# freewym/espresso

Measured on AMD Instinct MI355X. Metric: audio-hours/sec training (LibriSpeech Conformer-12 + CTC), higher is better.
Workload: dtype bf16; 1 GPU; LibriSpeech 960h Conformer-12 + CTC update step, <=26000 frames & <=24 utts per GPU, V=5004, on-GPU fbank+CMVN+SpecAugment, dropout 0.1, clip 2.0, Adam; parallelism=dp1

## Files before the change

espresso_amd/criterions/ctc_loss.py:

```python
import math

import torch

from .. import functional as F
from ..registry import register_criterion


@register_criterion("ctc_loss")
class CtcLossCriterion:
    def __init__(self, task, sentence_avg=True, zero_infinity=True, print_training_sample_interval=500):
        self.task = task
        d = task.target_dictionary
        if hasattr(task, "blank_symbol"):
            if task.blank_symbol is None:
                raise ValueError(f"{type(self).__name__} needs task.blank_symbol (task.criterion_name must name this criterion)")
            self.blank_idx = d.index(task.blank_symbol)
        else:
            self.blank_idx = d.bos()
        self.pad_idx = d.pad()
        self.eos_idx = d.eos()
        self.sentence_avg = sentence_avg
        self.zero_infinity = zero_infinity
        self.print_interval = print_training_sample_interval
        self.num_updates = -1
        self.epoch = 0

    def set_num_updates(self, num_updates):
        self.num_updates = num_updates

    def set_epoch(self, epoch):
        self.epoch = epoch

    def __call__(self, model, sample, reduce=True):
        return self.forward(model, sample, reduce)

    def forward(self, model, sample, reduce=True):
        net_output = model(**sample["net_input"], **({"epoch": self.epoch} if False else {}))
        input_lengths = net_output["src_lengths"][0]
        target = sample["target"]
        pad_mask = (target != self.pad_idx) & (target != self.eos_idx)
        target_lengths = pad_mask.sum(-1)
        lg = net_output.get("_logits_bt")
        if lg:
            logits = lg[0]
            B, Tp = net_output["encoder_padding_mask"][0].shape
        else:
            e = net_output["encoder_out"][0]
            Tp, B, V = e.shape
            logits = e.transpose(0, 1).reshape(B * Tp, V)
        nll, lprobs = F.ctc_loss(logits, target.to(torch.int32).contiguous(), input_lengths.to(torch.int32).contiguous(),
                                 target_lengths.to(torch.int32).contiguous(), B, Tp, blank=self.blank_idx,
                                 zero_infinity=self.zero_infinity)
        if self.zero_infinity:
            nll = torch.where(torch.isinf(nll), torch.zeros_like(nll), nll)
        loss = nll.sum()
        ntokens = sample["ntokens"] if "ntokens" in sample else int(target_lengths.sum())
        nsentences = target.size(0)
        sample_size = nsentences if self.sentence_avg else ntokens
        logging_output = {
            "loss": loss.detach(),
            "ntokens": ntokens,
            "nsentences": nsentences,
            "sample_size": sample_size,
        }
        return loss, sample_size, logging_output

    @staticmethod
    def reduce_metrics(logging_outputs):
        loss_sum = float(sum(float(l.get("loss", 0)) for l in logging_outputs))
        ntokens = sum(l.get("ntokens", 0) for l in logging_outputs)
        nsentences = sum(l.get("nsentences", 0) for l in logging_outputs)
        sample_size = sum(l.get("sample_size", 0) for l in logging_outputs)
        out = {"loss": loss_sum / max(sample_size, 1) / math.log(2), "ntokens": ntokens, "nsentences": nsentences,
               "sample_size": sample_size}
        if sample_size != ntokens:
            out["nll_loss"] = loss_sum / max(ntokens, 1) / math.log(2)
        return out

    @staticmethod
    def logging_outputs_can_be_summed():
        return True
```

espresso_amd/csrc/elementwise.hip:

```cpp
#include "common.h"
#include "espresso_amd.h"

namespace {

__global__ __launch_bounds__(256) void cast_f32_bf16_kernel(const float* __restrict__ src,
                                                            bf16_t* __restrict__ dst, long n) {
  const long stride = (long)gridDim.x * blockDim.x * 8;
  for (long i = ((long)blockIdx.x * blockDim.x + threadIdx.x) * 8; i < n; i += stride) {
    if (i + 8 <= n) {
      const float4 a = *reinterpret_cast<const float4*>(src + i);
      const float4 b = *reinterpret_cast<const float4*>(src + i + 4);
      uint4 u;
      u.x = pack_bf2(a.x, a.y);
      u.y = pack_bf2(a.z, a.w);
      u.z = pack_bf2(b.x, b.y);
      u.w = pack_bf2(b.z, b.w);
      *reinterpret_cast<uint4*>(dst + i) = u;
    } else {
      for (long j = i; j < n; ++j) dst[j] = f2bf(src[j]);
    }
  }
}

__global__ __launch_bounds__(256) void cast_f32_bf16_rows_kernel(const float* __restrict__ src, long ld_src, bf16_t* __restrict__ dst,
                                                                 long ld_dst, int N) {
  const long m = blockIdx.y;
  const float* s = src + m * ld_src;
  bf16_t* d = dst + m * ld_dst;
  const bool vec = (ld_src & 3) == 0 && (ld_dst & 7) == 0 && ((reinterpret_cast<uintptr_t>(src) | reinterpret_cast<uintptr_t>(dst)) & 15) == 0;
  for (int n = (blockIdx.x * 256 + threadIdx.x) * 8; n < ld_dst; n += gridDim.x * 256 * 8) {
    if (vec && n + 8 <= N) {
      const float4 a = *reinterpret_cast<const float4*>(s + n);
      const float4 b = *reinterpret_cast<const float4*>(s + n + 4);
      uint4 u;
      u.x = pack_bf2(a.x, a.y);
      u.y = pack_bf2(a.z, a.w);
      u.z = pack_bf2(b.x, b.y);
      u.w = pack_bf2(b.z, b.w);
      *reinterpret_cast<uint4*>(d + n) = u;
    } else {
      for (int j = n; j < n + 8 && j < ld_dst; ++j) d[j] = j < N ? f2bf(s[j]) : (bf16_t)0;
    }
  }
}

__global__ __launch_bounds__(256) void cast_bf16_f32_kernel(const bf16_t* __restrict__ src,
                                                            float* __restrict__ dst, long n) {
  const long stride = (long)gridDim.x * blockDim.x;
  for (long i = (long)blockIdx.x * blockDim.x + threadIdx.x; i < n; i += stride) dst[i] = bf2f(src[i]);
}

__global__ __launch_bounds__(256) void scale_dropout_kernel(const bf16_t* __restrict__ x,
                                                            const bf16_t* __restrict__ y,
                                                            bf16_t* __restrict__ out, long n, float a,
                                                            float b, uint64_t seed, uint32_t thr,
                                                            float inv_keep) {
  const long stride = (long)gridDim.x * blockDim.x * 8;
  for (long i = ((long)blockIdx.x * blockDim.x + threadIdx.x) * 8; i < n; i += stride) {
    if (i + 8 <= n) {
      const uint4 ux = *reinterpret_cast<const uint4*>(x + i);
      uint4 uy = make_uint4(0, 0, 0, 0);
      if (y) uy = *reinterpret_cast<const uint4*>(y + i);
      const uint32_t wx[4] = {ux.x, ux.y, ux.z, ux.w};
      const uint32_t wy[4] = {uy.x, uy.y, uy.z, uy.w};
      float o[8], k8[8];
      if (thr) ea_keep8(seed, (uint64_t)i, thr, inv_keep, k8);
#pragma unroll
      for (int e = 0; e < 8; ++e) {
        const float xv = (e & 1) ? __uint_as_float(wx[e >> 1] & 0xffff0000u) : __uint_as_float(wx[e >> 1] << 16);
        const float yv = (e & 1) ? __uint_as_float(wy[e >> 1] & 0xffff0000u) : __uint_as_float(wy[e >> 1] << 16);
        const float k = thr ? k8[e] : 1.f;
        o[e] = a * xv * k + b * yv;
      }
      uint4 u;
      u.x = pack_bf2(o[0], o[1]);
      u.y = pack_bf2(o[2], o[3]);
      u.z = pack_bf2(o[4], o[5]);
      u.w = pack_bf2(o[6], o[7]);
      *reinterpret_cast<uint4*>(out + i) = u;
    } else {
      for (long j = i; j < n; ++j) {
        float k = 1.f;
        if (thr) k = ea_keep(seed, (uint64_t)j, thr, inv_keep);
        out[j] = f2bf(a * bf2f(x[j]) * k + b * (y ? bf2f(y[j]) : 0.f));
      }
    }
  }
}

__global__ __launch_bounds__(256) void colsum_kernel(const bf16_t* __restrict__ X, float* __restrict__ out,
                                                     int M, int N, long ld, int rows_per_block) {
  __shared__ float sm[8][64];
  const int cx = threadIdx.x & 31, ry = threadIdx.x >> 5;
  const int c0 = blockIdx.x * 64 + cx * 2;
  const int r0 = blockIdx.y * rows_per_block;
  const int r1 = min(M, r0 + rows_per_block);
  float a0 = 0.f, a1 = 0.f;
  if (c0 + 1 < N && (ld & 1) == 0) {
    for (int r = r0 + ry; r < r1; r += 8) {
      const uint32_t w = *reinterpret_cast<const uint32_t*>(X + (long)r * ld + c0);
      a0 += __uint_as_float(w << 16);
      a1 += __uint_as_float(w & 0xffff0000u);
    }
  } else {
    for (int r = r0 + ry; r < r1; r += 8) {
      if (c0 < N) a0 += bf2f(X[(long)r * ld + c0]);
      if (c0 + 1 < N) a1 += bf2f(X[(long)r * ld + c0 + 1]);
    }
  }
  sm[ry][cx * 2] = a0;
  sm[ry][cx * 2 + 1] = a1;
  __syncthreads();
  if (threadIdx.x < 64) {
    float s = 0.f;
#pragma unroll
    for (int i = 0; i < 8; ++i) s += sm[i][threadIdx.x];
    const int c = blockIdx.x * 64 + threadIdx.x;
    if (c < N) atomicAdd(out + c, s);
  }
}

__global__ __launch_bounds__(256) void zero_rows_kernel(bf16_t* __restrict__ x, const uint8_t* __restrict__ row_zero,
                                                        int M, int C) {
  const int row = blockIdx.x;
  if (!row_zero[row]) return;
  for (int c = threadIdx.x; c < C; c += 256) x[(long)row * C + c] = 0;
}

__global__ __launch_bounds__(256) void embedding_fwd_kernel(const int* __restrict__ tok, const int* __restrict__ position,
                                                            const float* __restrict__ W, const float* __restrict__ pos,
                                                            bf16_t* __restrict__ out, int M, int C, float scale) {
  const int row = blockIdx.x * 4 + (threadIdx.x >> 6);
  if (row >= M) return;
  const float* w = W + (long)tok[row] * C;
  const float* pe = pos ? pos + (long)position[row] * C : nullptr;
  for (int c = (threadIdx.x & 63) * 2; c < C; c += 128) {
    float a = scale * w[c], b = scale * w[c + 1];
    if (pe) { a += pe[c]; b += pe[c + 1]; }
    *reinterpret_cast<uint32_t*>(out + (long)row * C + c) = pack_bf2(a, b);
  }
}
__global__ __launch_bounds__(256) void embedding_bwd_kernel(const int* __restrict__ tok, const bf16_t* __restrict__ dy,
                                                            float* __restrict__ dW, int M, int C, float scale, int pad_idx) {
  const int row = blockIdx.x * 4 + (threadIdx.x >> 6);
  if (row >= M) return;
  const int t = tok[row];
  if (t == pad_idx) return;
  float* w = dW + (long)t * C;
  for (int c = (threadIdx.x & 63); c < C; c += 64) atomicAdd(w + c, scale * bf2f(dy[(long)row * C + c]));
}

}

static inline int grid_for(long n, int per_thread) {
  long b = (n + 256L * per_thread - 1) / (256L * per_thread);
  if (b > 4096) b = 4096;
  if (b < 1) b = 1;
  return (int)b;
}

struct TransposeBatch {
  const bf16_t* src[8];
  bf16_t* dst[8];
  int rows[8], cols[8], tile0[9];
  int n;
};
__global__ __launch_bounds__(256) void transpose_batch_kernel(const TransposeBatch tb) {
  __shared__ bf16_t tile[64][66];
  int mi = 0;
#pragma unroll
  for (int i = 1; i < 8; ++i)
    if (i < tb.n && (int)blockIdx.x >= tb.tile0[i]) mi = i;
  const int R = tb.rows[mi], Cc = tb.cols[mi];
  const int tcols = (Cc + 63) / 64;
  const int t = blockIdx.x - tb.tile0[mi];
  const int r0 = (t / tcols) * 64, c0 = (t % tcols) * 64;
  const bf16_t* __restrict__ src = tb.src[mi];
  bf16_t* __restrict__ dst = tb.dst[mi];
  const int tx = threadIdx.x & 63, ty = threadIdx.x >> 6;
  for (int i = ty; i < 64; i += 4)
    if (r0 + i < R && c0 + tx < Cc) tile[i][tx] = src[(long)(r0 + i) * Cc + c0 + tx];
  __syncthreads();
  for (int i = ty; i < 64; i += 4)
    if (c0 + i < Cc && r0 + tx < R) dst[(long)(c0 + i) * R + r0 + tx] = tile[tx][i];
}

extern "C" int ea_transpose_bf16_batch(const void* const* src, void* const* dst, const int* rows, const int* cols, int n,
                                       hipStream_t stream) {
  if (n <= 0) return 0;
  if (n > 8) return -2;
  TransposeBatch tb;
  int tot = 0;
  for (int i = 0; i < 8; ++i) {
    tb.src[i] = i < n ? (const bf16_t*)src[i] : nullptr;
    tb.dst[i] = i < n ? (bf16_t*)dst[i] : nullptr;
    tb.rows[i] = i < n ? rows[i] : 0;
    tb.cols[i] = i < n ? cols[i] : 0;
    tb.tile0[i] = tot;
    if (i < n) tot += ((rows[i] + 63) / 64) * ((cols[i] + 63) / 64);
  }
  tb.tile0[8] = tot;
  tb.n = n;
  if (tot == 0) return 0;
  hipLaunchKernelGGL(transpose_batch_kernel, dim3(tot), dim3(256), 0, stream, tb);
  return EA_CHECK_LAUNCH();
}

extern "C" int ea_cast_f32_to_bf16(const float* src, void* dst, long n, hipStream_t stream) {
  if (n <= 0) return 0;
  hipLaunchKernelGGL(cast_f32_bf16_kernel, dim3(grid_for(n, 8)), dim3(256), 0, stream, src, (bf16_t*)dst, n);
  return EA_CHECK_LAUNCH();
}
extern "C" int ea_cast_f32_to_bf16_rows(const float* src, long ld_src, void* dst, long ld_dst, long M, int N, hipStream_t stream) {
  if (M <= 0 || N <= 0) return 0;
  if (ld_dst < N || ld_src < N || M > 65535) return -2;
  const int bx = (int)((ld_dst + 2047) / 2048);
  hipLaunchKernelGGL(cast_f32_bf16_rows_kernel, dim3(bx, (unsigned)M), dim3(256), 0, stream, src, ld_src, (bf16_t*)dst, ld_dst, N);
  return EA_CHECK_LAUNCH();
}
extern "C" int ea_cast_bf16_to_f32(const void* src, float* dst, long n, hipStream_t stream) {
  if (n <= 0) return 0;
  hipLaunchKernelGGL(cast_bf16_f32_kernel, dim3(grid_for(n, 1)), dim3(256), 0, stream, (const bf16_t*)src, dst, n);
  return EA_CHECK_LAUNCH();
}
extern "C" int ea_dropout_hash_host(uint64_t seed, uint64_t idx0, long n, uint32_t* out) {
  if (!out || n < 0) return -1;
  for (long i = 0; i < n; ++i) out[i] = ea_hash(seed, idx0 + (uint64_t)i);
  return 0;
}
extern "C" int ea_scale_dropout_bf16(const void* x, const void* y, void* out, long n, float a, float b,
                                     uint64_t seed, uint32_t thr, float inv_keep, hipStream_t stream) {
  if (n <= 0) return 0;
  hipLaunchKernelGGL(scale_dropout_kernel, dim3(grid_for(n, 8)), dim3(256), 0, stream, (const bf16_t*)x,
                     (const bf16_t*)y, (bf16_t*)out, n, a, b, seed, thr, inv_keep);
  return EA_CHECK_LAUNCH();
}
extern "C" int ea_colsum_bf16(const void* X, float* out, int M, int N, long ld, hipStream_t stream) {
  if (M <= 0 || N <= 0) return 0;
  int rpb = (M + 255) / 256;
  if (rpb < 64) rpb = 64;
  dim3 grid((N + 63) / 64, (M + rpb - 1) / rpb);
  hipLaunchKernelGGL(colsum_kernel, grid, dim3(256), 0, stream, (const bf16_t*)X, out, M, N, ld, rpb);
  return EA_CHECK_LAUNCH();
}
extern "C" int ea_zero_rows_bf16(void* x, const uint8_t* row_zero, int M, int C, hipStream_t stream) {
  if (M <= 0) return 0;
  hipLaunchKernelGGL(zero_rows_kernel, dim3(M), dim3(256), 0, stream, (bf16_t*)x, row_zero, M, C);
  return EA_CHECK_LAUNCH();
}

extern "C" int ea_embedding_fwd(const int* tokens, const int* positions, const float* W, const float* pos_table, void* out,
                                int M, int C, float scale, hipStream_t stream) {
  if (M <= 0) return 0;
  if (C % 2) return -2;
  hipLaunchKernelGGL(embedding_fwd_kernel, dim3((M + 3) / 4), dim3(256), 0, stream, tokens, positions, W, pos_table, (bf16_t*)out, M, C, scale);
  return EA_CHECK_LAUNCH();
}
extern "C" int ea_embedding_bwd(const int* tokens, const void* dy, float* dW, int M, int C, float scale, int pad_idx,
                                hipStream_t stream) {
  if (M <= 0) return 0;
  hipLaunchKernelGGL(embedding_bwd_kernel, dim3((M + 3) / 4), dim3(256), 0, stream, tokens, (const bf16_t*)dy, dW, M, C, scale, pad_idx);
  return EA_CHECK_LAUNCH();
}
```

espresso_amd/csrc/loss.hip:

```cpp
#include "common.h"
#include "espresso_amd.h"
#include "softmax_row.h"

namespace {

template <typename TIn>
__global__ __launch_bounds__(256) void log_softmax_kernel(const TIn* __restrict__ in, long ld_in,
                                                          float* __restrict__ out, int V) {
  __shared__ float sm[16];
  const long row = blockIdx.x;
  const TIn* x = in + row * ld_in;
  const float lse = log_softmax_row_lse<TIn, false>(x, V, sm);
  log_softmax_row_write<TIn, false>(x, V, lse, out + row * (long)V);
}

__device__ __forceinline__ int ctc_label(const int* tg, int s, int blank) { return (s & 1) ? tg[s >> 1] : blank; }

__global__ __launch_bounds__(256) void ctc_gather_kernel(const float* __restrict__ lprobs, const int* __restrict__ targets,
                                                         const int* __restrict__ in_len, const int* __restrict__ tgt_len,
                                                         float* __restrict__ G, int T, int V, int Lmax, int blank) {
  const int b = blockIdx.y, t = blockIdx.x;
  if (t >= in_len[b]) return;
  const int S = 2 * tgt_len[b] + 1, Smax = 2 * Lmax + 1;
  const float* lp = lprobs + ((long)b * T + t) * V;
  const int* tg = targets + (long)b * Lmax;
  float* g = G + ((long)b * T + t) * Smax;
  for (int s = threadIdx.x; s < S; s += blockDim.x) g[s] = lp[ctc_label(tg, s, blank)];
}

__global__ void ctc_scan_kernel(const float* __restrict__ G, const int* __restrict__ targets,
                                const int* __restrict__ in_len, const int* __restrict__ tgt_len,
                                float* __restrict__ A, float* __restrict__ Bt, float* __restrict__ nll_out,
                                int T, int Lmax, int blank, int SP) {
  extern __shared__ float sh[];
  const int b = blockIdx.x;
  const int Tb = in_len[b], L = tgt_len[b];
  const int S = 2 * L + 1, Smax = 2 * Lmax + 1;
  const int dir = blockIdx.y;
  const int s = threadIdx.x;
  float* buf0 = sh + 0 * (SP + 2) + (dir ? 0 : 2);
  float* buf1 = sh + 1 * (SP + 2) + (dir ? 0 : 2);
  const int* tg = targets + (long)b * Lmax;
  if (Tb <= 0) {
    if (threadIdx.x == 0 && dir == 0) nll_out[b] = (L == 0) ? 0.f : INFINITY;
    return;
  }
  bool skip = false;
  if (s < S) {
    if (!dir) { if ((s & 1) && s >= 2) skip = tg[s >> 1] != tg[(s >> 1) - 1]; }
    else      { if ((s & 1) && s + 2 < S) skip = tg[(s >> 1) + 1] != tg[s >> 1]; }
  }
  if (threadIdx.x < 2) {
    sh[0 * (SP + 2) + (dir ? SP : 0) + threadIdx.x] = -INFINITY;
    sh[1 * (SP + 2) + (dir ? SP : 0) + threadIdx.x] = -INFINITY;
  }
  const float* Gb = G + (long)b * T * Smax;
  float* Ob = (dir ? Bt : A) + (long)b * T * Smax;
  int t = dir ? Tb - 1 : 0;
  const int step = dir ? -1 : 1;
  {
    float v = -INFINITY;
    if (s < S) {
      const float lp = Gb[(long)t * Smax + s];
      if (!dir) { if (s == 0 || s == 1) v = lp; }
      else      { if (s == S - 1 || s == S - 2) v = lp; }
    }
    buf0[s] = v;
    if (s < S) Ob[(long)t * Smax + s] = v;
  }
  const long gstep = (long)step * Smax;
  const int sc = s < S ? s : (S - 1);
  const int so = s < S ? s : (S - 1);
  const float* g0 = Gb + (long)t * Smax + sc;
  auto row = [&](int it) { return g0 + (long)(it < Tb ? it : Tb - 1) * gstep; };
  float* op = Ob + (long)t * Smax + so;
  const bool live = s < S;
  __syncthreads();
  float* rd = buf0;
  float* wr = buf1;
  const int o1 = dir ? 1 : -1, o2 = dir ? 2 : -2;
  constexpr float LOG2E = 1.4426950408889634f, LN2 = 0.6931471805599453f;
  auto frame = [&](int it, float& q) {
    if (it >= Tb) return;
    const float lp = q;
    q = *row(it + 4);
    op += gstep;
    const float a0 = rd[s];
    const float a1 = rd[s + o1];
    const float a2 = skip ? rd[s + o2] : -INFINITY;
    const float m = fmaxf(a0, fmaxf(a1, a2));
    const float mm = m > -INFINITY ? m : 0.f;
    float v = mm + LN2 * __builtin_amdgcn_logf(__builtin_amdgcn_exp2f((a0 - mm) * LOG2E) + __builtin_amdgcn_exp2f((a1 - mm) * LOG2E) +
                                               __builtin_amdgcn_exp2f((a2 - mm) * LOG2E)) + lp;
    v = (live && m > -INFINITY) ? v : -INFINITY;
    if (live) *op = v;
    wr[s] = v;
    asm volatile("s_waitcnt lgkmcnt(0)" ::: "memory");
    __builtin_amdgcn_s_barrier();
    float* tmp = rd; rd = wr; wr = tmp;
  };
  float q1 = *row(1), q2 = *row(2), q3 = *row(3), q4 = *row(4);
  for (int it = 1; it < Tb; it += 4) {
    frame(it, q1);
    frame(it + 1, q2);
    frame(it + 2, q3);
    frame(it + 3, q4);
  }
  __syncthreads();
  if (threadIdx.x == 0 && dir == 0) {
    const float l1 = rd[S - 1];
    const float l2 = S >= 2 ? rd[S - 2] : -INFINITY;
    const float m = fmaxf(l1, l2);
    nll_out[b] = (m == -INFINITY) ? INFINITY : -(m + logf(expf(l1 - m) + expf(l2 - m)));
  }
}

template <typename TOut>
__global__ __launch_bounds__(256) void ctc_grad_kernel(const float* __restrict__ lprobs, const float* __restrict__ G,
                                                       const float* __restrict__ A, const float* __restrict__ Bt,
                                                       const float* __restrict__ nll, const int* __restrict__ targets,
                                                       const int* __restrict__ in_len, const int* __restrict__ tgt_len,
                                                       TOut* __restrict__ dlogits, long ld_out, int T, int V, int Lmax,
                                                       int blank, float scale, const float* __restrict__ scale_dev,
                                                       int zero_infinity) {
  extern __shared__ float post[];
  __shared__ float sm[16];
  const int b = blockIdx.y, t = blockIdx.x;
  TOut* out = dlogits + ((long)b * T + t) * ld_out;
  const float nl = nll[b];
  if (scale_dev) scale *= scale_dev[0];
  const bool dead = t >= in_len[b] || (zero_infinity && !(nl < INFINITY));
  for (int c = V + threadIdx.x; c < ld_out; c += 256) {
    if constexpr (sizeof(TOut) == 2) out[c] = 0; else out[c] = 0.f;
  }
  if (dead) {
    for (int c = threadIdx.x; c < V; c += 256) {
      if constexpr (sizeof(TOut) == 2) out[c] = 0; else out[c] = 0.f;
    }
    return;
  }
  for (int c = threadIdx.x; c < V; c += 256) post[c] = 0.f;
  __syncthreads();
  const int S = 2 * tgt_len[b] + 1, Smax = 2 * Lmax + 1;
  const long lo = ((long)b * T + t) * Smax;
  const int* tg = targets + (long)b * Lmax;
  float part = 0.f, blank_part = 0.f;
  for (int s = threadIdx.x; s < S; s += 256) {
    const float ab = A[lo + s] + Bt[lo + s];
    const float p = (ab == -INFINITY) ? 0.f : expf(ab + nl - G[lo + s]);
    part += p;
    if (s & 1) atomicAdd(&post[tg[s >> 1]], p); else blank_part += p;
  }
  const float sumpost = block_sum(part, sm);
  const float bsum = block_sum(blank_part, sm);
  if (threadIdx.x == 0) post[blank] += bsum;
  __syncthreads();
  const float* lp = lprobs + ((long)b * T + t) * V;
  for (int c = threadIdx.x; c < V; c += 256) {
    const float g = scale * (expf(lp[c]) * sumpost - post[c]);
    if constexpr (sizeof(TOut) == 2) out[c] = f2bf(g); else out[c] = g;
  }
}

template <typename TIn>
__global__ __launch_bounds__(256) void argmax_rows_kernel(const TIn* __restrict__ x, long ld, int V, int* __restrict__ best,
                                                          float* __restrict__ bestv) {
  __shared__ float sv[256];
  __shared__ int si[256];
  const long row = blockIdx.x;
  const TIn* r = x + row * ld;
  float mv = -INFINITY;
  int mi = 0x7fffffff;
  for (int c = threadIdx.x; c < V; c += 256) {
    float v;
    if constexpr (sizeof(TIn) == 2) v = bf2f(r[c]); else v = r[c];
    if (v > mv || (v == mv && c < mi)) { mv = v; mi = c; }
  }
  sv[threadIdx.x] = mv;
  si[threadIdx.x] = mi;
  __syncthreads();
  for (int s = 128; s > 0; s >>= 1) {
    if (threadIdx.x < s) {
      const float ov = sv[threadIdx.x + s];
      const int oi = si[threadIdx.x + s];
      if (ov > sv[threadIdx.x] || (ov == sv[threadIdx.x] && oi < si[threadIdx.x])) { sv[threadIdx.x] = ov; si[threadIdx.x] = oi; }
    }
    __syncthreads();
  }
  if (threadIdx.x == 0) { best[row] = si[0]; bestv[row] = sv[0]; }
}
__global__ void ctc_collapse_kernel(const int* __restrict__ best, const float* __restrict__ bestv, const int* __restrict__ in_len,
                                    int* __restrict__ tokens, int* __restrict__ align, int* __restrict__ out_len,
                                    float* __restrict__ score, int B, int T, int blank, int pad) {
  const int b = blockIdx.x * blockDim.x + threadIdx.x;
  if (b >= B) return;
  const int n = in_len[b];
  int u = 0, prev = -1;
  float s = 0.f;
  for (int t = 0; t < n; ++t) {
    const int k = best[(long)b * T + t];
    s += bestv[(long)b * T + t];
    if (k != blank && k != prev) {
      tokens[(long)b * T + u] = k;
      if (align) align[(long)b * T + u] = t;
      ++u;
    }
    prev = k;
  }
  for (int t = u; t < T; ++t) tokens[(long)b * T + t] = pad;
  out_len[b] = u;
  score[b] = s;
}

template <typename TIn, typename TOut>
__global__ __launch_bounds__(256) void lsce_kernel(const TIn* __restrict__ logits, long ld, const int* __restrict__ target,
                                                   float* __restrict__ out_loss, TOut* __restrict__ dlogits, long ld_out,
                                                   int V, int pad_idx, float eps, float scale, int smoothing,
                                                   const float* __restrict__ prior, int U) {
  __shared__ float sm[16];
  const long row = blockIdx.x;
  const TIn* x = logits + row * ld;
  const int tgt = target[row];
  TOut* dl = dlogits ? dlogits + row * ld_out : nullptr;
  if (tgt == pad_idx) {
    if (dl) for (int c = threadIdx.x; c < V; c += 256) { if constexpr (sizeof(TOut) == 2) dl[c] = 0; else dl[c] = 0.f; }
    return;
  }
  auto ld1 = [&](int c) -> float { if constexpr (sizeof(TIn) == 2) return bf2f(x[c]); else return x[c]; };
  float mx = -INFINITY, tot = 0.f;
  for (int c = threadIdx.x; c < V; c += 256) {
    const float v = ld1(c);
    mx = fmaxf(mx, v);
    tot += smoothing == 1 ? prior[c] * v : v;
  }
  mx = block_max(mx, sm);
  tot = block_sum(tot, sm);
  float s = 0.f;
  for (int c = threadIdx.x; c < V; c += 256) s += expf(ld1(c) - mx);
  s = block_sum(s, sm);
  const float lse = mx + logf(s);
  const float nll = lse - ld1(tgt);
  int nb[4] = {-1, -1, -1, -1};
  float nw[4] = {0.f, 0.f, 0.f, 0.f};
  float wsum = 1.f;
  float smooth, wn, we;
  if (smoothing == 2) {
    const int u = (int)(row % U);
    const int off[4] = {-2, -1, 1, 2};
    const float wt[4] = {2.f, 5.f, 5.f, 2.f};
    float z = 0.f;
#pragma unroll
    for (int k = 0; k < 4; ++k) {
      const int uu = u + off[k];
      if (uu < 0 || uu >= U) continue;
      const int t = target[row + off[k]];
      if (t == pad_idx) continue;
      nb[k] = t;
      nw[k] = wt[k];
      z += wt[k];
    }
    smooth = 0.f;
    if (z > 0.f) {
#pragma unroll
      for (int k = 0; k < 4; ++k)
        if (nb[k] >= 0) { nw[k] /= z; smooth += nw[k] * (lse - ld1(nb[k])); }
    } else {
      wsum = 0.f;
    }
    wn = 1.f - eps;
    we = eps;
  } else if (smoothing == 1) {
    smooth = lse - tot;
    wn = 1.f - eps;
    we = eps;
  } else {
    smooth = (float)V * lse - tot;
    we = eps / (float)(V - 1);
    wn = 1.f - eps - we;
    wsum = (float)V;
  }
  if (threadIdx.x == 0) {
    atomicAdd(out_loss + 0, wn * nll + we * smooth);
    atomicAdd(out_loss + 1, nll);
  }
  if (dl) {
    const float k = wn + we * wsum;
    for (int c = threadIdx.x; c < V; c += 256) {
      float g = expf(ld1(c) - lse) * k - (c == tgt ? wn : 0.f);
      if (smoothing == 0) g -= we;
      else if (smoothing == 1) g -= we * prior[c];
      else {
#pragma unroll
        for (int q = 0; q < 4; ++q) if (nb[q] == c) g -= we * nw[q];
      }
      g *= scale;
      if constexpr (sizeof(TOut) == 2) dl[c] = f2bf(g); else dl[c] = g;
    }
  }
}

}

extern "C" int ea_log_softmax_f32(const float* in, long ld_in, float* out, long M, int V, hipStream_t stream) {
  if (M <= 0) return 0;
  hipLaunchKernelGGL((log_softmax_kernel<float>), dim3((unsigned)M), dim3(256), 0, stream, in, ld_in, out, V);
  return EA_CHECK_LAUNCH();
}
extern "C" int ea_log_softmax_bf16(const void* in, long ld_in, float* out, long M, int V, hipStream_t stream) {
  if (M <= 0) return 0;
  hipLaunchKernelGGL((log_softmax_kernel<bf16_t>), dim3((unsigned)M), dim3(256), 0, stream, (const bf16_t*)in, ld_in, out, V);
  return EA_CHECK_LAUNCH();
}

extern "C" int ea_ctc_greedy_decode(const void* x, long ld, int x_bf16, const int* in_len, int* best ,
                                    float* bestv , int* tokens , int* align ,
                                    int* out_len, float* score, int B, int T, int V, int blank, int pad, hipStream_t stream) {
  if (B <= 0 || T <= 0) return 0;
  if (x_bf16)
    hipLaunchKernelGGL((argmax_rows_kernel<bf16_t>), dim3((unsigned)((long)B * T)), dim3(256), 0, stream, (const bf16_t*)x, ld, V, best, bestv);
  else
    hipLaunchKernelGGL((argmax_rows_kernel<float>), dim3((unsigned)((long)B * T)), dim3(256), 0, stream, (const float*)x, ld, V, best, bestv);
  hipLaunchKernelGGL(ctc_collapse_kernel, dim3((B + 63) / 64), dim3(64), 0, stream, best, bestv, in_len, tokens, align, out_len, score,
                     B, T, blank, pad);
  return EA_CHECK_LAUNCH();
}

extern "C" long ea_ctc_workspace_bytes(int B, int T, int Lmax) {
  return 3L * B * T * (2L * Lmax + 1) * (long)sizeof(float);
}

extern "C" int ea_ctc_loss(const float* lprobs, const int* targets, const int* in_len, const int* tgt_len,
                           float* nll , void* workspace, int B, int T, int V, int Lmax, int blank,
                           hipStream_t stream) {
  if (B <= 0) return 0;
  if (T <= 0 || V <= 0 || Lmax < 0) return -2;
  const int Smax = 2 * Lmax + 1;
  const int SP = ((Smax + 63) / 64) * 64;
  if (2 * SP > 1024) return -3;
  float* G = (float*)workspace;
  float* A = G + (long)B * T * Smax;
  float* Bt = A + (long)B * T * Smax;
  hipLaunchKernelGGL(ctc_gather_kernel, dim3(T, B), dim3(256), 0, stream, lprobs, targets, in_len, tgt_len, G, T, V,
                     Lmax, blank);
  hipLaunchKernelGGL(ctc_scan_kernel, dim3(B, 2), dim3(SP), (size_t)2 * (SP + 2) * sizeof(float), stream, G, targets,
                     in_len, tgt_len, A, Bt, nll, T, Lmax, blank, SP);
  return EA_CHECK_LAUNCH();
}

extern "C" int ea_ctc_grad(const float* lprobs, const void* workspace, const float* nll, const int* targets,
                           const int* in_len, const int* tgt_len, void* dlogits, long ld_out, int dlogits_bf16, int B,
                           int T, int V, int Lmax, int blank, float grad_scale, const float* grad_scale_dev,
                           int zero_infinity, hipStream_t stream) {
  if (B <= 0) return 0;
  const int Smax = 2 * Lmax + 1;
  const float* G = (const float*)workspace;
  const float* A = G + (long)B * T * Smax;
  const float* Bt = A + (long)B * T * Smax;
  if (dlogits_bf16)
    hipLaunchKernelGGL((ctc_grad_kernel<bf16_t>), dim3(T, B), dim3(256), (size_t)V * sizeof(float), stream, lprobs, G, A,
                       Bt, nll, targets, in_len, tgt_len, (bf16_t*)dlogits, ld_out, T, V, Lmax, blank, grad_scale,
                       grad_scale_dev, zero_infinity);
  else
    hipLaunchKernelGGL((ctc_grad_kernel<float>), dim3(T, B), dim3(256), (size_t)V * sizeof(float), stream, lprobs, G, A,
                       Bt, nll, targets, in_len, tgt_len, (float*)dlogits, ld_out, T, V, Lmax, blank, grad_scale,
                       grad_scale_dev, zero_infinity);
  return EA_CHECK_LAUNCH();
}

extern "C" int ea_label_smoothed_ce(const void* logits, long ld, int logits_bf16, const int* target,
                                    float* out_loss , void* dlogits, long ld_out, int dlogits_bf16, long M,
                                    int V, int pad_idx, float eps, float grad_scale, int smoothing, const float* prior,
                                    int tgt_len, hipStream_t stream) {
  if (M <= 0) return 0;
  if (smoothing < 0 || smoothing > 2 || (smoothing == 1 && !prior) || (smoothing == 2 && (tgt_len <= 0 || M % tgt_len))) return -2;
  dim3 g((unsigned)M), blk(256);
#define EA_LSCE(TI, TO)                                                                                               \
  hipLaunchKernelGGL((lsce_kernel<TI, TO>), g, blk, 0, stream, (const TI*)logits, ld, target, out_loss, (TO*)dlogits, ld_out, V, \
                     pad_idx, eps, grad_scale, smoothing, prior, tgt_len)
  if (logits_bf16) { if (dlogits_bf16 || !dlogits) EA_LSCE(bf16_t, bf16_t); else EA_LSCE(bf16_t, float); }
  else { if (dlogits_bf16 && dlogits) EA_LSCE(float, bf16_t); else EA_LSCE(float, float); }
#undef EA_LSCE
  return EA_CHECK_LAUNCH();
}
```

espresso_amd/functional.py:

```python
import collections

import ctypes
import os

import torch

from . import kernels as K

_seed_state = {"base": 0x5EED, "counter": 0}


def set_dropout_seed(seed: int):
    _seed_state["base"] = int(seed) & 0xFFFFFFFF
    _seed_state["counter"] = 0


_seed_trace = None


class trace_dropout_seeds:

    def __enter__(self):
        global _seed_trace
        self.prev, self.entries = _seed_trace, []
# ... 98 lines not shown
            zp["off"] = off + nbytes
            return zp["buf"][off: off + nbytes].view(dtype).view(shape)
    return torch.zeros(shape, dtype=dtype, device=device)


def _zeros_f32(n, like):
    return _pool_zeros((n,), torch.float32, like.device)


_DIRECT_GRADS = True


def set_direct_param_grads(on: bool) -> bool:
    global _DIRECT_GRADS
    old, _DIRECT_GRADS = _DIRECT_GRADS, bool(on)
    return old


_sink_scope = 0
_none_grad_hooks_ok = None


def _none_grad_hooks_fire() -> bool:
    global _none_grad_hooks_ok
    if _none_grad_hooks_ok is None:
        class _Probe(torch.autograd.Function):
            @staticmethod
            def forward(ctx, x, w):
                return x * 2

            @staticmethod
            def backward(ctx, dy):
                return dy * 2, None

        fired = []
        try:
            w = torch.nn.Parameter(torch.ones(2))
            w.grad = torch.zeros(2)
            w.register_post_accumulate_grad_hook(lambda p: fired.append(1))
            with torch.enable_grad():
                _Probe.apply(torch.ones(2, requires_grad=True), w).sum().backward()
        except Exception:
            fired = []
        _none_grad_hooks_ok = bool(fired)
    return _none_grad_hooks_ok


class accumulating_backward:

    def __enter__(self):
        global _sink_scope
        _none_grad_hooks_fire()
        _sink_scope += 1
        return self

    def __exit__(self, *exc):
        global _sink_scope
        _sink_scope -= 1
        if _sink_scope == 0:
            join_side_streams()
        return False


def _grad_sink(p, n=None):
    if not _DIRECT_GRADS or _sink_scope <= 0 or p is None or not getattr(p, "requires_grad", False):
        return None
    if not _none_grad_hooks_ok:
        return None
    if not p.is_leaf:
        return None
    g = p.grad
    if g is None or g.dtype != torch.float32 or not g.is_contiguous() or not g.is_cuda or (n is not None and g.numel() != n):
        return None
    return g.view(-1)




_side_streams = {}


def new_side_stream(device):
    st = torch.cuda.Stream(device=device)
    if os.environ.get("EA_SIDE_STREAM_PROBE", "1") == "0":
        _probe_log.append({"rejected": 0, "unprobed": True})
        return st
    from . import _lib

    cur = torch.cuda.current_stream(device)
    lib = _lib.lib()
    rejected, unprobed = 0, True
    with torch.cuda.device(device):
        for _ in range(7):
            if lib.ea_streams_share_queue(ctypes.c_void_p(cur.cuda_stream), ctypes.c_void_p(st.cuda_stream)) != 1:
                unprobed = False
                break
            rejected += 1
            st = torch.cuda.Stream(device=device)
    _probe_log.append({"rejected": rejected, "unprobed": unprobed})
    return st


_probe_log = []


def side_stream_probe_report():
    from . import _lib

    rej, unp = ctypes.c_int(-1), ctypes.c_int(0)
    have = _lib.lib().ea_side_stream_report(ctypes.byref(rej), ctypes.byref(unp))
    return {"layer_runtime": {"created": bool(have), "rejected": rej.value, "unprobed": bool(unp.value)},
            "python_streams": list(_probe_log)}


def _side_stream(device):
    key = str(device)
    st = _side_streams.get(key)
    if st is None:
        st = _side_streams[key] = new_side_stream(device)
    return st


_aux_streams = {}
_BRANCH_OVERLAP = True


def aux_stream(device, idx):
    key = (str(device), idx)
    st = _aux_streams.get(key)
    if st is None:
        st = _aux_streams[key] = new_side_stream(device)
    return st


def python_side_streams(device):
    key = str(torch.device(device))
    out = [st for k, st in _side_streams.items() if k == key]
    out += [st for (k, _), st in _aux_streams.items() if k == key]
    return out


def set_branch_overlap(on: bool) -> bool:
    global _BRANCH_OVERLAP
    old, _BRANCH_OVERLAP = _BRANCH_OVERLAP, bool(on)
    return old


def branch_overlap() -> bool:
    return _BRANCH_OVERLAP


class _Linear(torch.autograd.Function):
    @staticmethod
    def forward(ctx, x, w, b, w16, out_f32):
        M, Kin = x.shape
        N = w.shape[0]
        ld = _pad8(N)
        buf = _new((M, ld), torch.float32 if out_f32 else torch.bfloat16, x)
        K.gemm(x, w16, buf, M, N, Kin, lda=Kin, ldb=Kin, ldc=ld, bias=b)
        ctx.save_for_backward(x, w16)
        ctx.has_bias = b is not None
        ctx.params = (w, b)
        return buf if ld == N else buf[:, :N]

    @staticmethod
    def backward(ctx, dy):
        x, w16 = ctx.saved_tensors
        M, Kin = x.shape
        N = w16.shape[0]
        if dy.dtype != torch.bfloat16:
            if dy.stride(1) != 1:
                dy = dy.contiguous()
            dy = K.cast_f32_to_bf16_rows(dy, _pad8(N)) if M <= 65535 else K.cast_f32_to_bf16(dy.contiguous())
        if dy.stride(1) != 1 or dy.stride(0) % 8 != 0:
            dy = dy.contiguous()
        ld = dy.stride(0)
        pw, pb = ctx.params
        sW = _grad_sink(pw, N * Kin)
        sb = _grad_sink(pb, N) if ctx.has_bias else None
        if sW is not None and (sb is not None or not ctx.has_bias):
            side = _side_stream(dy.device) if (dy.is_cuda and 2.0 * M * N * Kin >= 4e9) else None
            if side is not None:
                cur = torch.cuda.current_stream(dy.device)
                side.wait_stream(cur)
                with torch.cuda.stream(side):
                    _wgrad(dy, x, M, N, Kin, ld_dy=ld, out=sW.view(N, Kin), accumulate=True)
                    if ctx.has_bias:
                        K.colsum(dy, sb, M, N, ld)
                dy.record_stream(side)
                x.record_stream(side)
                _side_pending[str(dy.device)] = True
            else:
                _wgrad(dy, x, M, N, Kin, ld_dy=ld, out=sW.view(N, Kin), accumulate=True)
                if ctx.has_bias:
                    K.colsum(dy, sb, M, N, ld)
            dW, db = None, None
        else:
            dW = _wgrad(dy, x, M, N, Kin, ld_dy=ld)
            db = None
            if ctx.has_bias:
                db = K.colsum(dy, _zeros_f32(N, dy), M, N, ld)
        dx = None
        if ctx.needs_input_grad[0]:
            dx = _new((M, Kin), torch.bfloat16, x)
            K.gemm(dy, w16, dx, M, Kin, N, lda=ld, ldb=Kin, ldc=Kin, b_kstrided=True)
        return dx, dW, db, None, None


def linear(x, w, b=None, out_f32=False):
    return _Linear.apply(x, w, b, bf16_weight(w), out_f32)


class _LayerNorm(torch.autograd.Function):
    @staticmethod
    def forward(ctx, x, g, b, eps, row_zero, drop_p, out_f32=False):
        seed = _next_seed("ln.out", drop_p) if drop_p > 0 else 0
        y, mean, rstd = K.layernorm_fwd(x, g, b, eps, row_zero, drop_p, seed, out_f32=out_f32)
        ctx.save_for_backward(x, g, mean, rstd, row_zero)
        ctx.drop = (drop_p, seed)
        ctx.params = (g, b)
        return y

    @staticmethod
    def backward(ctx, dy):
        x, g, mean, rstd, row_zero = ctx.saved_tensors
        C = x.shape[1]
        sg, sb = _grad_sink(ctx.params[0], C), _grad_sink(ctx.params[1], C)
        direct = sg is not None and sb is not None
        dg, db = (sg, sb) if direct else (_zeros_f32(C, x), _zeros_f32(C, x))
        dx = K.layernorm_bwd(x, dy.contiguous(), g, mean, rstd, dg, db, row_zero, ctx.drop[0], ctx.drop[1])
        if direct:
            return dx, None, None, None, None, None, None
        return dx, dg, db, None, None, None, None


def layer_norm(x, g, b, eps=1e-5, row_zero=None, drop_p=0.0, out_f32=False):
    return _LayerNorm.apply(x, g, b, eps, row_zero, drop_p, out_f32)


class _FFN(torch.autograd.Function):

    @staticmethod
    def forward(ctx, x, ln_g, ln_b, w1, b1, w2, b2, w1_16, w2_16, act, p_act, p_out, out_scale, eps):
        M, C = x.shape
        Fd = w1.shape[0]
        if ln_g is not None:
            xn, mean, rstd = K.layernorm_fwd(x, ln_g, ln_b, eps)
        else:
            xn, mean, rstd = x, None, None
        s1 = _next_seed("ffn.act", p_act) if p_act > 0 else 0
        s2 = _next_seed("ffn.out", p_out) if p_out > 0 else 0
        z = _new((M, Fd), torch.bfloat16, x)
        h = _new((M, Fd), torch.bfloat16, x)
        K.gemm(xn, w1_16, z, M, Fd, C, lda=C, ldb=C, ldc=Fd, bias=b1, act=act, C2=h, ldc2=Fd, drop_p=p_act, drop_seed=s1)
        y = _new((M, C), torch.bfloat16, x)
        K.gemm(h, w2_16, y, M, C, Fd, lda=Fd, ldb=Fd, ldc=C, bias=b2, drop_p=p_out, drop_seed=s2, out_scale=out_scale,
               resid=x, ldr=C)
        ctx.save_for_backward(x, ln_g, mean, rstd, xn, z, h, w1_16, w2_16)
        ctx.cfg = (act, p_act, p_out, out_scale, s1, s2)
        return y

    @staticmethod
    def backward(ctx, dy):
        x, ln_g, mean, rstd, xn, z, h, w1_16, w2_16 = ctx.saved_tensors
        act, p_act, p_out, out_scale, s1, s2 = ctx.cfg
        M, C = x.shape
        Fd = z.shape[1]
        dy = dy.contiguous()
        g2 = K.scale_dropout(dy, a=out_scale, drop_p=p_out, drop_seed=s2)
        dW2 = _wgrad(g2, h, M, C, Fd)
        db2 = K.colsum(g2, _zeros_f32(C, x), M, C, C)
        dz = _new((M, Fd), torch.bfloat16, x)
        K.gemm(g2, w2_16, dz, M, Fd, C, lda=C, ldb=Fd, ldc=Fd, b_kstrided=True, aux=z, ldaux=Fd, act=act, drop_p=p_act,
               drop_seed=s1)
        dW1 = _wgrad(dz, xn, M, Fd, C)
        db1 = K.colsum(dz, _zeros_f32(Fd, x), M, Fd, Fd)
        dxn = _new((M, C), torch.bfloat16, x)
        K.gemm(dz, w1_16, dxn, M, C, Fd, lda=Fd, ldb=C, ldc=C, b_kstrided=True)
        if ln_g is None:
            return dxn + dy, None, None, dW1, db1, dW2, db2, None, None, None, None, None, None, None
        dg, db = _zeros_f32(C, x), _zeros_f32(C, x)
        dx = K.layernorm_bwd(x, dxn, ln_g, mean, rstd, dg, db, dx_add=dy)
        return dx, dg, db, dW1, db1, dW2, db2, None, None, None, None, None, None, None


def ffn_module(x, ln_g, ln_b, w1, b1, w2, b2, act="silu", p_act=0.0, p_out=0.0, out_scale=0.5, eps=1e-5):
    return _FFN.apply(x, ln_g, ln_b, w1, b1, w2, b2, bf16_weight(w1), bf16_weight(w2), act, p_act, p_out, out_scale, eps)


def _pad8(n):
    return (n + 7) // 8 * 8


class _RelPosMHSA(torch.autograd.Function):

    @staticmethod
    def forward(ctx, x, ln_g, ln_b, wqkv, bqkv, wo, bo, u, v, wpos, wqkv16, wo16, wpos16, pe, key_len, attn_mask, B, T,
                H, p_attn, p_out, eps, pre_ln, causal=False):
        M, C = x.shape
        dh = C // H
        scaling = dh ** -0.5
        if pre_ln:
            xn, mean, rstd = K.layernorm_fwd(x, ln_g, ln_b, eps)
        else:
            xn, mean, rstd = x, None, None
        qkv = _new((M, 3 * C), torch.bfloat16, x)
        K.gemm(xn, wqkv16, qkv, M, 3 * C, C, lda=C, ldb=C, ldc=3 * C, bias=bqkv)
        relpos = pe is not None
        learned = relpos and wpos is None
        if learned:
            qu, _ = K.relpos_q_prep(qkv, 3 * C, None, None, M, C, scaling, want_qv=False)
            qv = qu
        else:
            qu, qv = K.relpos_q_prep(qkv, 3 * C, u if relpos else None, v if relpos else None, M, C, scaling, want_qv=relpos)
        Z = H * B
        Sp = _pad8(T)
        R = 2 * T - 1
        Rp = _pad8(R)
        pp = None
        if relpos:
            if learned:
                pp = K.cast_f32_to_bf16(pe.detach().contiguous())
            else:
                pp = _new((R, C), torch.bfloat16, x)
                K.gemm(pe, wpos16, pp, R, C, C, lda=C, ldb=C, ldc=C)
        sa = _next_seed("attn.probs", p_attn) if p_attn > 0 else 0
        fused = attn_mask is None and K.flash_attention_supported(dh, T, T, relpos)
        P = Pd = lse = bits = None
        if fused:
            o, lse, bits = K.flash_attention_fwd(qu, qv if relpos else None, qkv[:, C:], qkv[:, 2 * C:], pp, key_len, H, B, T, T, C,
                                                 3 * C, C, causal=causal, drop_p=p_attn, drop_seed=sa, want_bits=True)
        else:
            ac = _new((Z * T, Sp), torch.float32, x)
            K.gemm(qu, qkv, ac, T, T, dh, lda=C, ldb=3 * C, ldc=Sp, batch=Z, zdiv=B, sA=(dh, T * C), sB=(dh, T * 3 * C),
                   b_off=C, sC=(B * T * Sp, T * Sp))
            bd = None
            if relpos:
                bd = _new((Z * T, Rp), torch.float32, x)
                K.gemm(qv, pp, bd, T, R, dh, lda=C, ldb=C, ldc=Rp, batch=Z, zdiv=B, sA=(dh, T * C), sB=(dh, 0),
                       sC=(B * T * Rp, T * Rp))
            P, Pd = K.relpos_softmax_fwd(ac, bd, key_len, attn_mask, H, B, T, T, Sp, Rp, Sp, causal, p_attn, sa)
            del ac, bd
            o = _new((M, C), torch.bfloat16, x)
            K.gemm(Pd, qkv, o, T, dh, T, lda=Sp, ldb=3 * C, ldc=C, b_kstrided=True, batch=Z, zdiv=B, sA=(B * T * Sp, T * Sp),
                   sB=(dh, T * 3 * C), b_off=2 * C, sC=(dh, T * C))
        so = _next_seed("attn.out", p_out) if p_out > 0 else 0
        y = _new((M, C), torch.bfloat16, x)
        K.gemm(o, wo16, y, M, C, C, lda=C, ldb=C, ldc=C, bias=bo, drop_p=p_out, drop_seed=so, resid=x, ldr=C)
        ctx.save_for_backward(x, ln_g, mean, rstd, xn, qkv, qu, qv, pp, P, Pd, o, wqkv16, wo16, wpos16, pe, lse, key_len, bits)
        ctx.cfg = (B, T, H, p_attn, p_out, sa, so, pre_ln, relpos, learned, fused, causal)
        return y

    @staticmethod
    def backward(ctx, dy):
        (x, ln_g, mean, rstd, xn, qkv, qu, qv, pp, P, Pd, o, wqkv16, wo16, wpos16, pe, lse, key_len, bits) = ctx.saved_tensors
        B, T, H, p_attn, p_out, sa, so, pre_ln, relpos, learned, fused, causal = ctx.cfg
        M, C = x.shape
        dh = C // H
        scaling = dh ** -0.5
        Z = H * B
        Sp, R = _pad8(T), 2 * T - 1
        Rp = _pad8(R)
        dy = dy.contiguous()
        g = K.scale_dropout(dy, a=1.0, drop_p=p_out, drop_seed=so) if p_out > 0 else dy
        dWo = _wgrad(g, o, M, C, C)
        dbo = K.colsum(g, _zeros_f32(C, x), M, C, C)
        do = _new((M, C), torch.bfloat16, x)
        K.gemm(g, wo16, do, M, C, C, lda=C, ldb=C, ldc=C, b_kstrided=True)
        dqkv = _new((M, 3 * C), torch.bfloat16, x)
        t2 = dBD = None
        if fused:
            t1, t2, dBD = K.flash_attention_bwd(qu, qv if relpos else None, qkv[:, C:], qkv[:, 2 * C:], pp, key_len, o, do, lse,
                                                dqkv[:, C:], dqkv[:, 2 * C:], H, B, T, T, C, 3 * C, 3 * C, ldpp=C, causal=causal,
                                                scaling=scaling, drop_p=p_attn, drop_seed=sa, keep_bits=bits,
                                                dq=dqkv if relpos else None, lddq=3 * C)
        else:
            dPd = _new((Z * T, Sp), torch.float32, x)
            K.gemm(do, qkv, dPd, T, T, dh, lda=C, ldb=3 * C, ldc=Sp, batch=Z, zdiv=B, sA=(dh, T * C), sB=(dh, T * 3 * C),
                   b_off=2 * C, sC=(B * T * Sp, T * Sp))
            K.gemm(Pd, do, dqkv, T, dh, T, lda=Sp, ldb=C, ldc=3 * C, a_kstrided=True, b_kstrided=True, batch=Z, zdiv=B,
                   sA=(B * T * Sp, T * Sp), sB=(dh, T * C), sC=(dh, T * 3 * C), c_off=2 * C)
            dAC, dBD = K.relpos_softmax_bwd(P, dPd, H, B, T, T, Sp, Sp, Rp, want_bd=relpos, drop_p=p_attn, drop_seed=sa)
            del dPd
            K.gemm(dAC, qu, dqkv, T, dh, T, lda=Sp, ldb=C, ldc=3 * C, a_kstrided=True, b_kstrided=True, batch=Z, zdiv=B,
                   sA=(B * T * Sp, T * Sp), sB=(dh, T * C), sC=(dh, T * 3 * C), c_off=C)
            t1 = _new((M, C), torch.bfloat16, x)
            K.gemm(dAC, qkv, t1, T, dh, T, lda=Sp, ldb=3 * C, ldc=C, b_kstrided=True, batch=Z, zdiv=B, sA=(B * T * Sp, T * Sp),
                   sB=(dh, T * 3 * C), b_off=C, sC=(dh, T * C), alpha=scaling)
            if relpos:
                t2 = _new((M, C), torch.bfloat16, x)
                K.gemm(dBD, pp, t2, T, dh, R, lda=Rp, ldb=C, ldc=C, b_kstrided=True, batch=Z, zdiv=B, sA=(B * T * Rp, T * Rp),
                       sB=(dh, 0), sC=(dh, T * C), alpha=scaling)
        du = dv = dWpos = dpe = None
        if relpos:
            dpp32 = _new((R, C), torch.float32, x)
            K.gemm(dBD, qv, dpp32, R, dh, B * T, lda=Rp, ldb=C, ldc=C, a_kstrided=True, b_kstrided=True, batch=H, zdiv=1,
                   sA=(B * T * Rp, 0), sB=(dh, 0), sC=(dh, 0), splitk=_auto_splitk(((R + 127) // 128) * H, B * T))
            if learned:
                dpe = dpp32
            else:
                dWpos = _wgrad(K.cast_f32_to_bf16(dpp32), pe, R, C, C)
                du = K.colsum(t1, _zeros_f32(C, x), M, C, C)
                dv = K.colsum(t2, _zeros_f32(C, x), M, C, C)
            if not fused:
                K.add2_strided(t1, C, t2, C, dqkv, 3 * C, M, C)
        else:
            K.add2_strided(t1, C, torch.zeros_like(t1), C, dqkv, 3 * C, M, C)
        dWqkv = _wgrad(dqkv, xn, M, 3 * C, C)
        dbqkv = K.colsum(dqkv, _zeros_f32(3 * C, x), M, 3 * C, 3 * C)
        dxn = _new((M, C), torch.bfloat16, x)
        K.gemm(dqkv, wqkv16, dxn, M, C, 3 * C, lda=3 * C, ldb=C, ldc=C, b_kstrided=True)
        if pre_ln:
            dg, db = _zeros_f32(C, x), _zeros_f32(C, x)
            dx = K.layernorm_bwd(x, dxn, ln_g, mean, rstd, dg, db, dx_add=dy)
        else:
            dg = db = None
            dx = K.scale_dropout(dxn, a=1.0, y=dy, b=1.0)
        return (dx, dg, db, dWqkv, dbqkv, dWo, dbo, du, dv, dWpos, None, None, None, dpe) + (None,) * 10


def relpos_mhsa(x, ln_g, ln_b, wqkv, bqkv, wo, bo, u, v, wpos, pe, key_len, attn_mask, B, T, H, p_attn=0.0, p_out=0.0,
                eps=1e-5, pre_ln=True, wqkv16=None, causal=False):
    return _RelPosMHSA.apply(
        x, ln_g, ln_b, wqkv, bqkv, wo, bo, u, v, wpos, wqkv16 if wqkv16 is not None else bf16_weight(wqkv),
        bf16_weight(wo), bf16_weight(wpos) if wpos is not None else None, pe, key_len, attn_mask, B, T, H, p_attn, p_out,
        eps, pre_ln, causal)


class _ConvModule(torch.autograd.Function):

    @staticmethod
    def forward(ctx, x, ln_g, ln_b, wpw1, wdw, bn_g, bn_b, wpw2, wpw1_16, wpw2_16, running_mean, running_var, B, T, KW,
                p_out, eps, bn_eps, bn_momentum, training, causal=False):
        M, C = x.shape
        xn, mean, rstd = K.layernorm_fwd(x, ln_g, ln_b, eps)
        Y = _new((M, 2 * C), torch.bfloat16, x)
        K.gemm(xn, wpw1_16, Y, M, 2 * C, C, lda=C, ldb=C, ldc=2 * C)
        wdw2 = wdw.detach().reshape(C, KW).contiguous()
        stats = torch.zeros(2 * C, dtype=torch.float64, device=x.device) if training else None
        U, Zt = K.glu_dwconv_fwd(Y, wdw2, B, T, C, KW, stats, causal=causal)
        if training:
            mr = K.bn_finalize(stats, C, M, bn_eps, bn_momentum, running_mean, running_var)
        else:
            mr = K.bn_from_running(running_mean, running_var, bn_eps)
        Hh = K.bn_act_fwd(Zt, mr, bn_g, bn_b, "silu")
        so = _next_seed("conv.out", p_out) if p_out > 0 else 0
        y = _new((M, C), torch.bfloat16, x)
        K.gemm(Hh, wpw2_16, y, M, C, C, lda=C, ldb=C, ldc=C, drop_p=p_out, drop_seed=so, resid=x, ldr=C)
        ctx.save_for_backward(x, ln_g, mean, rstd, xn, Y, U, Zt, mr, Hh, bn_g, bn_b, wdw2, wpw1_16, wpw2_16)
        ctx.cfg = (B, T, KW, p_out, so, training, causal)
        ctx.wdw_shape = wdw.shape
        return y

    @staticmethod
    def backward(ctx, dy):
        (x, ln_g, mean, rstd, xn, Y, U, Zt, mr, Hh, bn_g, bn_b, wdw2, wpw1_16, wpw2_16) = ctx.saved_tensors
        B, T, KW, p_out, so, training, causal = ctx.cfg
        M, C = x.shape
        dy = dy.contiguous()
        g = K.scale_dropout(dy, a=1.0, drop_p=p_out, drop_seed=so) if p_out > 0 else dy
        dWpw2 = _wgrad(g, Hh, M, C, C)
        dH = _new((M, C), torch.bfloat16, x)
        K.gemm(g, wpw2_16, dH, M, C, C, lda=C, ldb=C, ldc=C, b_kstrided=True)
        dbn_g, dbn_b = _zeros_f32(C, x), _zeros_f32(C, x)
        dZ = K.bn_act_bwd(Zt, dH, mr, bn_g, bn_b, dbn_g, dbn_b, "silu", training)
        dwdw = _zeros_f32(C * KW, x)
        dY = K.glu_dwconv_bwd(dZ, Y, U, wdw2, dwdw, B, T, C, KW, causal=causal)
        dWpw1 = _wgrad(dY, xn, M, 2 * C, C)
        dxn = _new((M, C), torch.bfloat16, x)
        K.gemm(dY, wpw1_16, dxn, M, C, 2 * C, lda=2 * C, ldb=C, ldc=C, b_kstrided=True)
        dg, db = _zeros_f32(C, x), _zeros_f32(C, x)
        dx = K.layernorm_bwd(x, dxn, ln_g, mean, rstd, dg, db, dx_add=dy)
        return (dx, dg, db, dWpw1.view(2 * C, C, 1), dwdw.view(ctx.wdw_shape), dbn_g, dbn_b, dWpw2.view(C, C, 1)) + (None,) * 13


def conv_module(x, ln_g, ln_b, wpw1, wdw, bn_g, bn_b, wpw2, running_mean, running_var, B, T, p_out=0.0, eps=1e-5,
                bn_eps=1e-5, bn_momentum=0.1, training=True, causal=False):
    C = x.shape[1]
    KW = wdw.shape[-1]
    return _ConvModule.apply(x, ln_g, ln_b, wpw1, wdw, bn_g, bn_b, wpw2, bf16_weight(wpw1).view(2 * C, C),
                             bf16_weight(wpw2).view(C, C), running_mean, running_var, B, T, KW, p_out, eps, bn_eps,
                             bn_momentum, training, bool(causal))


class _CTCLoss(torch.autograd.Function):

    @staticmethod
    def forward(ctx, logits, targets, in_len, tgt_len, B, T, blank, zero_infinity):
        M, V = logits.shape
        assert M == B * T
        if logits.stride(1) != 1:
            logits = logits.contiguous()
        Lmax = targets.shape[1]
        lprobs = K.log_softmax(logits, M, V, logits.stride(0))
        nll, ws = K.ctc_loss_fwd(lprobs, targets, in_len, tgt_len, B, T, V, Lmax, blank)
        ctx.save_for_backward(lprobs, ws, nll, targets, in_len, tgt_len)
        ctx.cfg = (B, T, V, Lmax, blank, zero_infinity, logits.dtype)
        ctx.mark_non_differentiable(lprobs)
        return nll, lprobs

    @staticmethod
    def backward(ctx, dnll, _dlp):
        lprobs, ws, nll, targets, in_len, tgt_len = ctx.saved_tensors
        B, T, V, Lmax, blank, zero_infinity, dt = ctx.cfg
        scale_dev = dnll.float().contiguous()
        bf = dt == torch.bfloat16
        ld = _pad8(V) if bf else V
        dl = K.ctc_loss_grad(lprobs, ws, nll, targets, in_len, tgt_len, B, T, V, Lmax, blank, ld_out=ld, grad_bf16=bf,
                             grad_scale=1.0, grad_scale_dev=scale_dev, zero_infinity=zero_infinity)
        return (dl if ld == V else dl[:, :V]), None, None, None, None, None, None, None


def ctc_loss(logits, targets, in_len, tgt_len, B, T, blank=0, zero_infinity=True):
    return _CTCLoss.apply(logits, targets, in_len, tgt_len, B, T, blank, zero_infinity)


class _LabelSmoothedCE(torch.autograd.Function):

    @staticmethod
    def forward(ctx, logits, target, pad_idx, eps, smoothing="uniform", prior=None, tgt_len=0):
        M, V = logits.shape
        if logits.stride(1) != 1:
            logits = logits.contiguous()
        out, _ = K.label_smoothed_ce(logits, logits.stride(0), target, M, V, pad_idx, eps, want_grad=False, smoothing=smoothing,
                                     prior=prior, tgt_len=tgt_len)
        ctx.save_for_backward(logits, target, prior)
        ctx.cfg = (pad_idx, eps, smoothing, tgt_len)
        return out[0], out[1]

    @staticmethod
    def backward(ctx, dloss, _dnll):
        logits, target, prior = ctx.saved_tensors
        pad_idx, eps, smoothing, tgt_len = ctx.cfg
        M, V = logits.shape
        bf = logits.dtype == torch.bfloat16
        _, dl = K.label_smoothed_ce(logits, logits.stride(0), target, M, V, pad_idx, eps, want_grad=True, grad_bf16=bf,
                                    grad_ld=_pad8(V) if bf else V, smoothing=smoothing, prior=prior, tgt_len=tgt_len)
        g = dl if dl.shape[1] == V else dl[:, :V]
        return g * dloss.to(g.dtype), None, None, None, None, None, None


def label_smoothed_ce(logits, target, pad_idx, eps, smoothing="uniform", prior=None, tgt_len=0):
    return _LabelSmoothedCE.apply(logits, target, pad_idx, eps, smoothing, prior, tgt_len)


_CONV_IGEMM = True


_CONV1_FUSED_BWD = True


def set_conv1_fused_backward(on: bool) -> bool:
    global _CONV1_FUSED_BWD
    old, _CONV1_FUSED_BWD = _CONV1_FUSED_BWD, bool(on)
    return old


def set_conv_implicit_gemm(on: bool):
    global _CONV_IGEMM
    _CONV_IGEMM = bool(on)


def _conv_igemm_ok(cin, cout, sy, sx):
    return _CONV_IGEMM and cin in (64, 128) and cout in (64, 128) and sy in (1, 2) and sx in (1, 2)


class _ConvSubsample(torch.autograd.Function):

    @staticmethod
    def forward(ctx, X, row_zero, strides, bufs, p_drop, training, bn_eps, bn_momentum, after_first_layer, *params):
        B, T, F = X.shape
        L = len(params) // 4
        saved = []
        cfgs = []
        A = None
        Tc, Fc, Cc = T, F, 1
        for i in range(L):
            w, b, g, beta = params[4 * i: 4 * i + 4]
            rm, rv = bufs[2 * i], bufs[2 * i + 1]
            sy, sx = strides[i]
            Co = w.shape[0]
            To, Fo = (Tc - 1) // sy + 1, (Fc - 1) // sx + 1
            stats = _pool_zeros((2 * Co,), torch.float64, X.device) if training else None
            if i == 0:
                assert w.shape[1] == 1 and tuple(w.shape[2:]) == (3, 3)
                Zi = K.conv1_fwd(X, w.detach().reshape(Co, 9).contiguous(), b, B, Tc, Fc, Co, sy, sx, stats)
                col, w16 = None, None
            elif _conv_igemm_ok(Cc, Co, sy, sx):
                w16 = K.cast_f32_to_bf16(w.detach().permute(0, 2, 3, 1).reshape(Co, 9 * Cc).contiguous())
                Zi = K.conv3x3_fwd(A, w16, b, B, Tc, Fc, Cc, Co, sy, sx, stats=stats)
                col = A
            else:
                col = K.im2col3x3(A, B, Tc, Fc, Cc, sy, sx)
                w16 = K.cast_f32_to_bf16(w.detach().permute(0, 2, 3, 1).reshape(Co, 9 * Cc).contiguous())
                Zi = _new((B * To * Fo, Co), torch.bfloat16, X)
                K.gemm(col, w16, Zi, B * To * Fo, Co, 9 * Cc, lda=9 * Cc, ldb=9 * Cc, ldc=Co, bias=b)
                if training:
                    K.colstats(Zi, stats)
            n = B * To * Fo
            mr = K.bn_finalize(stats, Co, n, bn_eps, bn_momentum, rm, rv) if training else K.bn_from_running(rm, rv, bn_eps)
            A = K.bn_act_fwd(Zi, mr, g, beta, "relu")
            if i == 0 and after_first_layer is not None:
                after_first_layer()
            saved += [Zi, mr, col, w16, g, beta]
            cfgs.append((Tc, Fc, Cc, To, Fo, Co, sy, sx))
            Tc, Fc, Cc = To, Fo, Co
        out = A.view(B * Tc, Fc * Cc)
        seed = _next_seed("subsample.out", p_drop) if (training and p_drop > 0) else 0
        if seed:
            out = K.scale_dropout(out, a=1.0, drop_p=p_drop, drop_seed=seed)
        if row_zero is not None:
            K.zero_rows(out, row_zero)
        ctx.save_for_backward(X, row_zero, *[t for t in saved if t is not None])
        ctx.layout = [[t is not None for t in saved[6 * i: 6 * i + 6]] for i in range(L)]
        ctx.cfg = (B, cfgs, p_drop, seed, training, [tuple(p.shape) for p in params[0::4]])
        ctx.igemm = [i > 0 and _conv_igemm_ok(cfgs[i][2], cfgs[i][5], cfgs[i][6], cfgs[i][7]) for i in range(L)]
        ctx.weights = [params[4 * i] for i in range(L)]
        ctx.params = list(params)
        return out

    @staticmethod
    def backward(ctx, dout):
        X, row_zero, *flat = ctx.saved_tensors
        B, cfgs, p_drop, seed, training, wshapes = ctx.cfg
        L = len(cfgs)
        it = iter(flat)
        per = []
        for i in range(L):
            per.append([next(it) if has else None for has in ctx.layout[i]])
        dout = dout.contiguous()
        if seed:
            dout = K.scale_dropout(dout, a=1.0, drop_p=p_drop, drop_seed=seed)
        elif row_zero is not None:
            dout = dout.clone()
        if row_zero is not None:
            K.zero_rows(dout, row_zero)
        grads = [None] * (4 * L)
        Tc, Fc, Cc, To, Fo, Co, sy, sx = cfgs[-1]
        dA = dout.view(B * To * Fo, Co)
        cur = torch.cuda.current_stream(X.device)
        side = _side_stream(X.device)
        keep = []
        for i in range(L - 1, -1, -1):
            Zi, mr, col, w16, g, beta = per[i]
            Tc, Fc, Cc, To, Fo, Co, sy, sx = cfgs[i]
            pw, pb, pg, pbe = ctx.params[4 * i: 4 * i + 4]
            sg, sbe = (_grad_sink(pg, Co), _grad_sink(pbe, Co)) if training else (None, None)
            if sg is not None and sbe is not None:
                dg, dbeta = sg, sbe
            else:
                sg = sbe = None
                dg, dbeta = _zeros_f32(Co, X), _zeros_f32(Co, X)
            if i == 0 and Co % 64 == 0 and _CONV1_FUSED_BWD:
                sW, sb = _grad_sink(pw, Co * 9), _grad_sink(pb, Co)
                if sW is not None and sb is not None:
                    db, dW = sb, sW
                else:
                    sW = None
                    db, dW = _zeros_f32(Co, X), _zeros_f32(Co * 9, X)
                K.conv1_bn_bwd(X, Zi, dA, mr, g, beta, dg, dbeta, dW, db, B, Tc, Fc, Co, sy, sx, "relu", training)
                if sW is None:
                    grads[0], grads[1] = dW.view(wshapes[0]), db
                if sg is None:
                    grads[2], grads[3] = dg, dbeta
                continue
            dZ = K.bn_act_bwd(Zi, dA, mr, g, beta, dg, dbeta, "relu", training)
            keep.append(dZ)
# ... 1348 lines not shown
```

espresso_amd/kernels.py:

```python
import ctypes
from typing import Optional

import torch

from . import _lib
from ._lib import EaGemmParams, check

ACT_NONE, ACT_RELU, ACT_SILU = 0, 1, 2
_ACT = {None: 0, "none": 0, "relu": 1, "silu": 2, "swish": 2}


def _stream():
    return ctypes.c_void_p(torch._C._cuda_getCurrentRawStream(torch._C._cuda_getDevice()))


def _p(t: Optional[torch.Tensor]):
    if t is None:
        return None
    if not t.is_cuda:
        raise RuntimeError("espresso_amd kernels need device tensors (no CPU path)")
    return ctypes.c_void_p(t.data_ptr())


def drop_params(p: float):
# ... 225 lines not shown
                                          C, _p(lse), _p(D), _p(t1), _p(t2), C, _p(dBD), Rp, _p(dk), _p(dv), lddkv, H, B, T, S,
                                          dh, int(causal), scaling, drop_seed, thr, scale, _p(keep_bits), _p(dq), lddq,
                                          _stream()),
        "ea_flash_attention_bwd",
    )
    return t1, t2, dBD


def relpos_softmax_bwd(P, dPd, H, B, T, S, ld_p, ld_dp, ld_bd, want_bd=True, drop_p=0.0, drop_seed=0):
    dAC = torch.empty(H * B * T, ld_p, dtype=torch.bfloat16, device=P.device)
    dBD = torch.empty(H * B * T, ld_bd, dtype=torch.bfloat16, device=P.device) if want_bd else None
    thr, scale = drop_params(drop_p)
    check(
        _lib.lib().ea_relpos_softmax_bwd(_p(P), _p(dPd), _p(dAC), _p(dBD), H, B, T, S, ld_p, ld_dp, ld_bd, drop_seed,
                                         thr, scale, _stream()),
        "ea_relpos_softmax_bwd",
    )
    return dAC, dBD


def add2_strided(a, lda, b, ldb, out, ldo, M, C, out_off=0):
    check(
        _lib.lib().ea_add2_strided_bf16(_p(a), lda, _p(b), ldb, ctypes.c_void_p(out.data_ptr() + 2 * out_off), ldo, M,
                                        C, _stream()),
        "ea_add2_strided_bf16",
    )
    return out


def glu_dwconv_fwd(Y, w, B, T, C, KW, stats, causal=False):
    U = torch.empty(B * T, C, dtype=torch.bfloat16, device=Y.device)
    Z = torch.empty(B * T, C, dtype=torch.bfloat16, device=Y.device)
    name = "ea_glu_dwconv_causal_fwd" if causal else "ea_glu_dwconv_fwd"
    check(getattr(_lib.lib(), name)(_p(Y), _p(w), _p(U), _p(Z), _p(stats), B, T, C, KW, _stream()), name)
    return U, Z


def bn_finalize(stats, C, n, eps, momentum, running_mean=None, running_var=None):
    mean_rstd = torch.empty(2, C, dtype=torch.float32, device=stats.device)
    check(_lib.lib().ea_bn_finalize(_p(stats), _p(mean_rstd), _p(running_mean), _p(running_var), C, float(n), eps,
                                    momentum, _stream()), "ea_bn_finalize")
    return mean_rstd


def bn_from_running(running_mean, running_var, eps):
    C = running_mean.numel()
    mean_rstd = torch.empty(2, C, dtype=torch.float32, device=running_mean.device)
    check(_lib.lib().ea_bn_from_running(_p(running_mean), _p(running_var), _p(mean_rstd), C, eps, _stream()),
          "ea_bn_from_running")
    return mean_rstd


def bn_act_fwd(Z, mean_rstd, gamma, beta, act):
    M, C = Z.shape
    H = torch.empty_like(Z)
    check(_lib.lib().ea_bn_act_fwd(_p(Z), _p(mean_rstd), _p(gamma), _p(beta), _p(H), M, C, _ACT[act], _stream()),
          "ea_bn_act_fwd")
    return H


def conv1_bn_bwd(X, Z, dH, mean_rstd, gamma, beta, dgamma, dbeta, dW, dbias, B, T, F, CO, sy, sx, act, training=True):
    from . import functional as _F

    red = _F._pool_zeros((2, CO), torch.float32, Z.device)
    check(_lib.lib().ea_conv1_bn_bwd(_p(X), _p(Z), _p(dH), _p(mean_rstd), _p(gamma), _p(beta), _p(red), _p(dgamma), _p(dbeta), _p(dW),
                                     _p(dbias), B, T, F, CO, sy, sx, _ACT[act], int(training), _stream()), "ea_conv1_bn_bwd")


def bn_act_bwd(Z, dH, mean_rstd, gamma, beta, dgamma, dbeta, act, training=True):
    M, C = Z.shape
    from . import functional as _F

    red = _F._pool_zeros((2, C), torch.float32, Z.device)
    dZ = torch.empty_like(Z)
    check(
        _lib.lib().ea_bn_act_bwd(_p(Z), _p(dH), _p(mean_rstd), _p(gamma), _p(beta), _p(red), _p(dZ), _p(dgamma),
                                 _p(dbeta), M, C, _ACT[act], int(training), _stream()),
        "ea_bn_act_bwd",
    )
    return dZ


def glu_dwconv_bwd(dZ, Y, U, w, dw, B, T, C, KW, causal=False):
    dY = torch.empty(B * T, 2 * C, dtype=torch.bfloat16, device=Y.device)
    ws = torch.empty(int(_lib.lib().ea_dwconv_wgrad_workspace_bytes(B, T, C, KW)), dtype=torch.uint8, device=Y.device)
    name = "ea_glu_dwconv_causal_bwd" if causal else "ea_glu_dwconv_bwd"
    check(getattr(_lib.lib(), name)(_p(dZ), _p(Y), _p(U), _p(w), _p(dY), _p(dw), _p(ws), B, T, C, KW, _stream()), name)
    return dY


def conv1_fwd(X, W, bias, B, T, F, CO, sy, sx, stats):
    To, Fo = (T - 1) // sy + 1, (F - 1) // sx + 1
    Z = torch.empty(B * To * Fo, CO, dtype=torch.bfloat16, device=X.device)
    check(_lib.lib().ea_conv1_fwd(_p(X), _p(W), _p(bias), _p(Z), _p(stats), B, T, F, CO, sy, sx, _stream()),
          "ea_conv1_fwd")
    return Z


def conv1_wgrad(X, dZ, dW, dbias, B, T, F, CO, sy, sx):
    check(_lib.lib().ea_conv1_wgrad(_p(X), _p(dZ), _p(dW), _p(dbias), B, T, F, CO, sy, sx, _stream()), "ea_conv1_wgrad")


def conv3x3_fwd(X, W16, bias, B, T, F, Cin, Cout, sy, sx, stats=None):
    To, Fo = (T - 1) // sy + 1, (F - 1) // sx + 1
    Z = torch.empty((B * To * Fo, Cout), dtype=torch.bfloat16, device=X.device)
    check(_lib.lib().ea_conv3x3_fwd(_p(X), _p(W16), _p(bias), _p(Z), _p(stats), B, T, F, Cin, Cout, sy, sx, _stream()), "ea_conv3x3_fwd")
    return Z


def conv3x3_dgrad(dZ, Wd16, B, T, F, Cin, Cout, sy, sx):
    dX = torch.empty((B * T * F, Cin), dtype=torch.bfloat16, device=dZ.device)
    check(_lib.lib().ea_conv3x3_dgrad(_p(dZ), _p(Wd16), _p(dX), B, T, F, Cin, Cout, sy, sx, _stream()), "ea_conv3x3_dgrad")
    return dX


def conv3x3_wgrad(X, dZ, dW, B, T, F, Cin, Cout, sy, sx, param_layout=False):
    lib = _lib.lib()
    nb = lib.ea_conv3x3_wgrad_workspace_bytes(B, T, F, Cin, Cout, sy, sx)
    ws = torch.empty(nb, dtype=torch.uint8, device=X.device)
    fn = lib.ea_conv3x3_wgrad_param_layout if param_layout else lib.ea_conv3x3_wgrad
    check(fn(_p(X), _p(dZ), _p(dW), _p(ws), B, T, F, Cin, Cout, sy, sx, _stream()), "ea_conv3x3_wgrad")
    return dW


def im2col3x3(A, B, T, F, C, sy, sx):
    To, Fo = (T - 1) // sy + 1, (F - 1) // sx + 1
    col = torch.empty(B * To * Fo, 9 * C, dtype=torch.bfloat16, device=A.device)
    check(_lib.lib().ea_im2col3x3(_p(A), _p(col), B, T, F, C, sy, sx, _stream()), "ea_im2col3x3")
    return col


def col2im3x3(dcol, B, T, F, C, sy, sx):
    dA = torch.empty(B * T * F, C, dtype=torch.bfloat16, device=dcol.device)
    check(_lib.lib().ea_col2im3x3(_p(dcol), _p(dA), B, T, F, C, sy, sx, _stream()), "ea_col2im3x3")
    return dA


def colstats(X, stats):
    M, C = X.shape
    check(_lib.lib().ea_colstats_bf16(_p(X), _p(stats), M, C, _stream()), "ea_colstats_bf16")
    return stats


def log_softmax(x, M, V, ld):
    out = torch.empty(M, V, dtype=torch.float32, device=x.device)
    if x.dtype == torch.float32:
        check(_lib.lib().ea_log_softmax_f32(_p(x), ld, _p(out), M, V, _stream()), "ea_log_softmax_f32")
    else:
        assert x.dtype == torch.bfloat16
        check(_lib.lib().ea_log_softmax_bf16(_p(x), ld, _p(out), M, V, _stream()), "ea_log_softmax_bf16")
    return out


def ctc_loss_fwd(lprobs, targets, in_len, tgt_len, B, T, V, Lmax, blank):
    assert lprobs.dtype == torch.float32 and lprobs.is_contiguous()
    assert targets.dtype == torch.int32 and in_len.dtype == torch.int32 and tgt_len.dtype == torch.int32
    dev = lprobs.device
    nll = torch.empty(B, dtype=torch.float32, device=dev)
    ws = torch.empty(int(_lib.lib().ea_ctc_workspace_bytes(B, T, Lmax)), dtype=torch.uint8, device=dev)
    check(
        _lib.lib().ea_ctc_loss(_p(lprobs), _p(targets), _p(in_len), _p(tgt_len), _p(nll), _p(ws), B, T, V, Lmax, blank,
                               _stream()),
        "ea_ctc_loss",
    )
    return nll, ws


def ctc_loss_grad(lprobs, ws, nll, targets, in_len, tgt_len, B, T, V, Lmax, blank, ld_out=None, grad_bf16=True,
                  grad_scale=1.0, grad_scale_dev=None, zero_infinity=True):
    ld_out = V if ld_out is None else ld_out
    dl = torch.empty(B * T, ld_out, dtype=torch.bfloat16 if grad_bf16 else torch.float32, device=lprobs.device)
    check(
        _lib.lib().ea_ctc_grad(_p(lprobs), _p(ws), _p(nll), _p(targets), _p(in_len), _p(tgt_len), _p(dl), ld_out,
                               int(grad_bf16), B, T, V, Lmax, blank, grad_scale, _p(grad_scale_dev),
                               int(zero_infinity), _stream()),
        "ea_ctc_grad",
    )
    return dl


SMOOTHING = {"uniform": 0, "unigram": 1, "temporal": 2}


def label_smoothed_ce(logits, ld, target, M, V, pad_idx, eps, want_grad=True, grad_bf16=True, grad_scale=1.0,
                      grad_ld=None, smoothing="uniform", prior=None, tgt_len=0):
    assert target.dtype == torch.int32
    dev = logits.device
    out = torch.zeros(2, dtype=torch.float32, device=dev)
    dl = None
    grad_ld = V if grad_ld is None else grad_ld
    if want_grad:
        dl = torch.zeros(M, grad_ld, dtype=torch.bfloat16 if grad_bf16 else torch.float32, device=dev)
    check(
        _lib.lib().ea_label_smoothed_ce(_p(logits), ld, int(logits.dtype == torch.bfloat16), _p(target), _p(out),
                                        _p(dl), grad_ld, int(grad_bf16), M, V, pad_idx, eps, grad_scale, SMOOTHING[smoothing],
                                        _p(prior), tgt_len, _stream()),
        "ea_label_smoothed_ce",
    )
    return out, dl


def fbank_batch(wav, offsets, B, tables, cmvn_mean, cmvn_std, Tmax, nmel=80, frame_len=400, frame_shift=160,
                preemph=0.97, log_floor=1.1920928955078125e-07, want_sum=True):
    dev = wav.device
    feat = torch.empty(B, Tmax, nmel, dtype=torch.float32, device=dev)
    utt_sum = torch.zeros(B, dtype=torch.float32, device=dev) if want_sum else None
    out_len = torch.empty(B, dtype=torch.int32, device=dev)
    assert wav.dtype in (torch.float32, torch.int16)
    fn = _lib.lib().ea_fbank_batch if wav.dtype == torch.float32 else _lib.lib().ea_fbank_batch_i16
    check(
        fn(_p(wav), _p(offsets), B, _p(tables["window"]), _p(tables["twiddle"]), _p(tables["mel_start"]), _p(tables["mel_len"]),
           _p(tables["mel_woff"]), _p(tables["mel_w"]), _p(cmvn_mean), _p(cmvn_std), _p(feat), _p(utt_sum), _p(out_len), Tmax, nmel,
           frame_len, frame_shift, preemph, log_floor, _stream()),
        "ea_fbank_batch",
    )
    return feat, out_len, utt_sum


def feature_stats(feat, lengths, acc):
    B, Tmax, nmel = feat.shape
    assert acc.dtype == torch.float64 and acc.numel() == 2 * nmel + 1 and feat.dtype == torch.float32 and feat.is_contiguous()
    check(_lib.lib().ea_feature_stats(_p(feat), _p(lengths), _p(acc), B, Tmax, nmel, _stream()), "ea_feature_stats")
    return acc


def specaugment(feat, lengths, utt_sum, fmask, tmask, use_mean=True, mask_value=0.0):
    B, Tmax, nmel = feat.shape
    nf = fmask.shape[1] if fmask is not None else 0
    nt = tmask.shape[1] if tmask is not None else 0
    check(
        _lib.lib().ea_specaugment(_p(feat), _p(lengths), _p(utt_sum), _p(fmask), _p(tmask), nf, nt, B, Tmax, nmel,
                                  int(use_mean), mask_value, _stream()),
        "ea_specaugment",
    )
    return feat


def grad_sumsq(g, out):
    check(_lib.lib().ea_grad_sumsq(_p(g), g.numel(), _p(out), _stream()), "ea_grad_sumsq")
    return out


def clip_coef(sumsq, pre_scale, max_norm, coef, denom_dev=None):
    check(_lib.lib().ea_clip_coef(_p(sumsq), pre_scale, _p(denom_dev), max_norm, _p(coef), _stream()), "ea_clip_coef")
    return coef


def adam_step(p, g, m, v, p_bf16, coef, lr, beta1, beta2, eps, weight_decay, step, zero_grad=True):
    check(
        _lib.lib().ea_adam_step(_p(p), _p(g), _p(m), _p(v), _p(p_bf16), p.numel(), _p(coef), lr, beta1, beta2, eps,
                                weight_decay, step, int(zero_grad), _stream()),
        "ea_adam_step",
    )


def clip_coef_clear(sumsq, pre_scale, max_norm, coef, denom_dev=None):
    check(_lib.lib().ea_clip_coef_clear(_p(sumsq), pre_scale, _p(denom_dev), max_norm, _p(coef), _stream()), "ea_clip_coef_clear")
    return coef


def adam_step_capped(p, g, m, v, p_bf16, coef, lr, beta1, beta2, eps, weight_decay, step, max_blocks, stream, zero_grad=True):
    check(
        _lib.lib().ea_adam_step_capped(_p(p), _p(g), _p(m), _p(v), _p(p_bf16), p.numel(), _p(coef), lr, beta1, beta2, eps,
                                       weight_decay, step, int(zero_grad), int(max_blocks), ctypes.c_void_p(stream.cuda_stream)),
        "ea_adam_step_capped",
    )


def ctc_greedy_decode(x, in_len, B, T, V, blank, pad, ld=None, want_align=True):
    dev = x.device
    ld = x.stride(0) if ld is None else ld
    best = torch.empty(B * T, dtype=torch.int32, device=dev)
    bestv = torch.empty(B * T, dtype=torch.float32, device=dev)
    tokens = torch.empty(B, T, dtype=torch.int32, device=dev)
    align = torch.zeros(B, T, dtype=torch.int32, device=dev) if want_align else None
    out_len = torch.empty(B, dtype=torch.int32, device=dev)
    score = torch.empty(B, dtype=torch.float32, device=dev)
    check(
        _lib.lib().ea_ctc_greedy_decode(_p(x), ld, int(x.dtype == torch.bfloat16), _p(in_len), _p(best), _p(bestv), _p(tokens),
                                        _p(align), _p(out_len), _p(score), B, T, V, blank, pad, _stream()),
        "ea_ctc_greedy_decode",
    )
    return tokens, out_len, score, align


def _finish_outputs(n, nbest, max_u, device):
    return (torch.empty(n, nbest, max_u, dtype=torch.int32, device=device), torch.empty(n, nbest, dtype=torch.int32, device=device),
            torch.empty(n, nbest, dtype=torch.float32, device=device), torch.empty(n, dtype=torch.int32, device=device))


def _partial_outputs(n, max_u, device):
    return (torch.empty(n, max_u, dtype=torch.int32, device=device), torch.empty(n, dtype=torch.int32, device=device),
            torch.empty(n, dtype=torch.float32, device=device), torch.empty(n, dtype=torch.int32, device=device))


def _stream_state(bytes_fn, max_streams, max_frames, beam, device):
    nbytes = int(bytes_fn(max_frames, beam))
    assert nbytes > 0 and max_streams >= 1
    return torch.zeros(max_streams, nbytes, dtype=torch.uint8, device=device), nbytes


def _check_stream_state(state, bytes_fn, max_frames, beam):
    assert state.dtype == torch.uint8 and state.is_contiguous() and state.dim() == 2
    assert state.shape[1] == bytes_fn(max_frames, beam)


def _check_rnnt_step_args(logits, out, lm_rows, N, V, lm_no_blank):
    assert logits.dtype == torch.float32 and logits.dim() == 2 and logits.stride(1) == 1 and logits.shape[0] == N and logits.shape[1] >= V
    parent, token, keep = out
    assert parent.numel() == token.numel() == keep.numel() == N
    assert parent.dtype == token.dtype == torch.int32 and keep.dtype == torch.uint8
    if lm_rows is not None:
        assert lm_rows.dtype == torch.float32 and lm_rows.stride(1) == 1 and lm_rows.shape == (N, V - 1 if lm_no_blank else V)
    return parent, token, keep


def ctc_prefix_beam_workspace(B, T, beam, device):
    return torch.empty(int(_lib.lib().ea_ctc_prefix_beam_workspace_bytes(B, T, beam)), dtype=torch.uint8, device=device)
# ... 1163 lines not shown
```

espresso_amd/models/transformer/speech_transformer_encoder_model.py:

```python
import os

import torch
import torch.nn as nn

from ... import functional as F
from ... import kernels as K
from ...modules.conformer_layer import ConformerWithRelativePositionalEmbeddingEncoderLayer
from ...modules.params import LayerNormParams, LinearParams
from ...modules.learned_relative_positional_embedding import LearnedRelativePositionalEmbedding
from ...modules.sinusoidal_relative_positional_embedding import SinusoidalRelativePositionalEmbedding
from ...modules.speech_convolutions import ConvBNReLU
from ...modules.transformer_layer import TransformerWithRelativePositionalEmbeddingEncoderLayer
from ...registry import register_model, register_model_architecture
from ...tools import utils as speech_utils
from .speech_transformer_config import DEFAULT_MAX_SOURCE_POSITIONS, SpeechTransformerConfig

_LOGITS_F32 = os.environ.get("EA_LOGITS_F32", "0") == "1"


class AbsolutePositionTable(nn.Module):

    def __init__(self, num_embeddings, dim):
        super().__init__()
        self.weight = nn.Parameter(torch.empty(num_embeddings, dim))
        nn.init.normal_(self.weight, mean=0, std=dim ** -0.5)
        nn.init.constant_(self.weight[0], 0)


class SpeechTransformerEncoderBase(nn.Module):
    def __init__(self, cfg, pre_encoder=None, input_size=83):
        super().__init__()
        self.cfg = cfg
        self.register_buffer("version", torch.Tensor([3]))
        d = cfg.encoder.embed_dim
        self.embed_dim = d
        self.max_source_positions = cfg.max_source_positions
        self.pre_encoder = pre_encoder
        self.fc0 = LinearParams(input_size, d) if input_size != d else None
        self.embed_scale = 1.0 if (cfg.no_scale_embedding or self.fc0 is not None) else d ** 0.5
        self.embed_positions = None
        self.abs_positions = not cfg.encoder.relative_positional_embeddings and not cfg.no_token_positional_embeddings
        if self.abs_positions and cfg.encoder.learned_pos:
            n = int(self.output_lengths(cfg.max_source_positions)) if pre_encoder is not None else cfg.max_source_positions
            self.embed_positions = AbsolutePositionTable(n + 1, d)
        self._sin_table = None
        self.layernorm_embedding = LayerNormParams(d) if cfg.layernorm_embedding else None
        nl = cfg.encoder.layers
        if not cfg.encoder.relative_positional_embeddings:
            rels = [None] * nl
        elif cfg.encoder.learned_pos:
            dim = d // cfg.encoder.attention_heads if getattr(cfg.encoder, "share_learned_relative_positional_embeddings_across_heads", False) else d
            size = int(self.output_lengths(cfg.max_source_positions)) if pre_encoder is not None else cfg.max_source_positions
            if getattr(cfg.encoder, "share_learned_relative_positional_embeddings_across_layers", False):
                rels = [LearnedRelativePositionalEmbedding(dim, max_size=size)] * nl
            else:
                rels = [LearnedRelativePositionalEmbedding(dim, max_size=size) for _ in range(nl)]
        else:
            rels = [SinusoidalRelativePositionalEmbedding(d)] * nl
        self.rel_pos_embed = [rels[0]]
        if getattr(cfg.encoder, "depthwise_conv_causal", False) and cfg.encoder.layer_type != "conformer":
            raise ValueError(f"encoder.depthwise_conv_causal needs encoder.layer_type: conformer (got {cfg.encoder.layer_type}: "
                             "only the conformer layer has a depthwise convolution)")
        if cfg.encoder.layer_type == "conformer":
            layer_cls = ConformerWithRelativePositionalEmbeddingEncoderLayer
        elif cfg.encoder.layer_type == "transformer":
            layer_cls = TransformerWithRelativePositionalEmbeddingEncoderLayer
        else:
            raise NotImplementedError(cfg.encoder.layer_type)
        self.layers = nn.ModuleList([layer_cls(cfg, positional_embedding=rels[i]) for i in range(nl)])
        self.num_layers = len(self.layers)
        if cfg.encoder.normalize_before and cfg.encoder.layer_type != "conformer":
            self.layer_norm = LayerNormParams(d)
        else:
            self.layer_norm = None
        self.transformer_context = speech_utils.eval_str_nested_list_or_tuple(cfg.encoder.transformer_context, type=int)
        self.num_updates = 0
        self.pending_update = None
        if pre_encoder is not None:
            pre_encoder.after_first_layer = self.start_pending_update

    def set_num_updates(self, num_updates):
        self.num_updates = num_updates

    def start_pending_update(self):
        if self.pending_update is not None:
            self.pending_update.start()

    def early_modules(self):
        return [self.pre_encoder, self.fc0, self.embed_positions, self.layernorm_embedding]

    def output_lengths(self, in_lengths):
        return in_lengths if self.pre_encoder is None else self.pre_encoder.output_lengths(in_lengths)

    def get_attn_mask(self, max_len, device, in_lengths=None):
        if self.cfg.encoder.chunk_size > 0:
            from ...data.data_utils import numpy_seed

            with numpy_seed(self.num_updates):
                vis = speech_utils.chunk_streaming_mask(in_lengths, self.cfg.encoder.chunk_size,
                                                        left_window=self.cfg.encoder.chunk_left_window,
                                                        right_window=self.cfg.encoder.chunk_right_window,
                                                        always_partial_in_last=not self.training)
            return torch.zeros(max_len, max_len, device=device).masked_fill(~vis.to(device), -1e8).contiguous()
        tc = self.transformer_context
        if tc is None or (tc[0] is None and tc[1] is None):
            return None
        ones = torch.ones(max_len, max_len, dtype=torch.bool, device=device)
        if tc[0] is None:
            m = ones.triu(tc[1] + 1)
        elif tc[1] is None:
            m = ones.tril(-tc[0] - 1)
        else:
            m = ones.triu(tc[1] + 1) | ones.tril(-tc[0] - 1)
        return torch.zeros(max_len, max_len, device=device).masked_fill(m, -1e8).contiguous()

    def _count_batchnorm_forward(self, device):
        flat = getattr(self, "_bn_counters", None)
        mods = getattr(self, "_bn_counter_mods", None)
        ok = (flat is not None and flat.device == device and len(mods) > 0
              and mods[0].num_batches_tracked.data_ptr() == flat.data_ptr())
        if not ok:
            owners = ([self.pre_encoder] if self.pre_encoder is not None else []) + [l for l in self.layers if hasattr(l, "conv_module")]
            mods = list(self.pre_encoder.batchnorms) if self.pre_encoder is not None else []
            mods += [l.conv_module.batch_norm for l in self.layers if hasattr(l, "conv_module")]
            if not mods:
                self._bn_counters, self._bn_counter_mods = None, []
                return
            flat = torch.stack([m.num_batches_tracked.detach().to(device).long().reshape(()) for m in mods])
            for i, m in enumerate(mods):
                m._buffers["num_batches_tracked"] = flat[i]
            for o in owners:
                o._counters_managed = True
            self._bn_counters, self._bn_counter_mods = flat, mods
        flat.add_(1)

    def _add_positions(self, x, padding_mask):
        B, Tp = padding_mask.shape
        valid = (~padding_mask).to(torch.int64)
        pos = (torch.cumsum(valid, dim=1) * valid).reshape(-1)
        if not self.abs_positions:
            table = torch.zeros(1, self.embed_dim, device=x.device)
            pos = torch.zeros_like(pos)
        elif self.embed_positions is not None:
            table = self.embed_positions.weight
        else:
            if self._sin_table is None or self._sin_table.shape[0] < Tp + 1 or self._sin_table.device != x.device:
                from .speech_transformer_base import sinusoidal_positional_table

                self._sin_table = sinusoidal_positional_table(max(Tp + 1, 1024), self.embed_dim, 0).to(x.device)
            table = self._sin_table
        return F.add_positions(x, table, pos, self.embed_scale)

    def _fc0_weight(self):
        w = self.fc0.weight
        C = self.pre_encoder.out_channels[-1]
        Fp = w.shape[1] // C
        return w.view(w.shape[0], C, Fp).permute(0, 2, 1).reshape(w.shape[0], Fp * C)

    def encode(self, src_tokens, src_lengths, return_all_hiddens=False):
        cfg = self.cfg
        tr = self.training
        B = src_tokens.shape[0]
        p = cfg.dropout if tr else 0.0
        if tr and float(getattr(cfg.encoder, "layerdrop", 0.0) or 0.0) == 0.0 and src_tokens.is_cuda:
            self._count_batchnorm_forward(src_tokens.device)
        x, x_lengths, padding_mask, row_zero = self.pre_encoder(src_tokens, src_lengths, p_drop=p if self.fc0 is not None else 0.0)
        Tp = padding_mask.shape[1]
        if self.fc0 is not None:
            x = F.linear(x, self._fc0_weight(), self.fc0.bias)
        if self.abs_positions or self.embed_scale != 1.0:
            x = self._add_positions(x, padding_mask)
        if self.layernorm_embedding is not None:
            x = F.layer_norm(x, self.layernorm_embedding.weight, self.layernorm_embedding.bias, row_zero=row_zero, drop_p=p)
        else:
            if p > 0:
                x = F.dropout(x, p)
            if row_zero is not None:
                x = F.zero_rows(x, row_zero)
        key_len = x_lengths.to(torch.int32).contiguous()
        attn_mask = self.get_attn_mask(Tp, x.device, in_lengths=x_lengths)
        states = [x] if return_all_hiddens else []
        ld = float(getattr(cfg.encoder, "layerdrop", 0.0) or 0.0)
        keep = torch.empty(len(self.layers)).uniform_() > ld if (tr and ld > 0) else None
        wt_event = None
        if tr and torch.is_grad_enabled() and x.is_cuda:
            native = [l for i, l in enumerate(self.layers) if (keep is None or bool(keep[i])) and _native_conformer(l)]
            if native:
                wt_event = F.refresh_layer_transposes(native, B, Tp)
        if self.pending_update is not None:
            self.pending_update.wait(torch.cuda.current_stream(x.device))
            self.pending_update = None
        kept = [l for i, l in enumerate(self.layers) if keep is None or bool(keep[i])]
        if (not return_all_hiddens and x.is_cuda and all(_native_conformer(l) for l in kept) and F.conformer_stack_supported(kept, x)):
            l0 = kept[0]
            c0 = l0.cfg
            x = F.conformer_stack_native(x, kept, key_len, attn_mask, l0.positional_embedding[0].table(Tp, x.device), B, Tp,
                                         c0.dropout if tr else 0.0, c0.activation_dropout if tr else 0.0,
                                         c0.attention_dropout if tr else 0.0, tr)
            if tr:
                for l in kept:
                    if not getattr(l, "_counters_managed", False):
                        l.conv_module.batch_norm.num_batches_tracked += 1
            kept = []
        for i, layer in enumerate(kept):        kept = [l for i, l in enumerate(self.layers) if keep is None or bool(keep[i])]
        for i, layer in enumerate(kept):
            nxt = kept[i + 1] if i + 1 < len(kept) else None
            if nxt is not None and not return_all_hiddens and x.is_cuda and _native_conformer(layer) and _native_conformer(nxt):
                x = layer(x, B, Tp, key_len=key_len, attn_mask=attn_mask, chain_next=nxt)
            else:
                x = layer(x, B, Tp, key_len=key_len, attn_mask=attn_mask)
            if return_all_hiddens:
                states.append(x)
        if wt_event is not None:
            torch.cuda.current_stream(x.device).wait_event(wt_event)
        if self.layer_norm is not None:
            x = F.layer_norm(x, self.layer_norm.weight, self.layer_norm.bias)
        return x, x_lengths, padding_mask, B, Tp, states

    def forward(self, src_tokens, src_lengths, return_all_hiddens=False):
        x, x_lengths, padding_mask, B, Tp, states = self.encode(src_tokens, src_lengths, return_all_hiddens)
        C = x.shape[1]
        return {
            "encoder_out": [x.view(B, Tp, C).transpose(0, 1)],
            "encoder_padding_mask": [padding_mask],
            "encoder_embedding": [],
            "encoder_states": [s.view(B, Tp, C).transpose(0, 1) for s in states],
            "fc_results": [],
            "src_tokens": [],
            "src_lengths": [x_lengths],
            "_x_bt": [x],
        }

    def max_positions(self):
        return self.max_source_positions

    def reorder_encoder_out(self, encoder_out, new_order):
        out = dict(encoder_out)
        out["encoder_out"] = [e.index_select(1, new_order) for e in encoder_out["encoder_out"]]
        out["encoder_padding_mask"] = [m.index_select(0, new_order) for m in encoder_out["encoder_padding_mask"]]
        out["src_lengths"] = [l.index_select(0, new_order) for l in encoder_out["src_lengths"]]
        out["encoder_states"] = [s.index_select(1, new_order) for s in encoder_out["encoder_states"]]
        out.pop("_x_bt", None)
        return out


def _native_conformer(layer) -> bool:
    pe = getattr(layer, "positional_embedding", [None])[0]
    return (hasattr(layer, "conv_module") and getattr(layer, "use_native_runtime", False) and pe is not None
            and not getattr(pe, "learnable", False))


class SpeechTransformerEncoderForPrediction(SpeechTransformerEncoderBase):

    def __init__(self, cfg, pre_encoder=None, input_size=83, vocab_size=None):
        super().__init__(cfg, pre_encoder=pre_encoder, input_size=input_size)
        self.fc_out = LinearParams(cfg.encoder.embed_dim, vocab_size) if vocab_size is not None else None

    def forward(self, src_tokens, src_lengths, return_all_hiddens=False):
        out = super().forward(src_tokens, src_lengths, return_all_hiddens=return_all_hiddens)
        if self.fc_out is not None:
            x = out.pop("_x_bt")[0]
            B, Tp = out["encoder_padding_mask"][0].shape
            logits = F.linear(x, self.fc_out.weight, self.fc_out.bias, out_f32=_LOGITS_F32)
            V = logits.shape[1]
            out["encoder_out"] = [logits.view(B, Tp, V).transpose(0, 1)]
            out["_logits_bt"] = [logits]
        return out


@register_model("speech_transformer_encoder_model", dataclass=SpeechTransformerConfig)
class SpeechTransformerEncoderModel(nn.Module):
    config_class = SpeechTransformerConfig

    def __init__(self, cfg, encoder):
        super().__init__()
        self.cfg = cfg
        self.encoder = encoder
        self.num_updates = 0

    @classmethod
    def build_model(cls, cfg, task):
        if cfg.max_source_positions is None:
            cfg.max_source_positions = DEFAULT_MAX_SOURCE_POSITIONS
        ev = speech_utils.eval_str_nested_list_or_tuple
        out_channels = ev(cfg.encoder.conv_channels, type=int)
        kernel_sizes = ev(cfg.encoder.conv_kernel_sizes, type=int)
        strides = ev(cfg.encoder.conv_strides, type=int)
        assert task.feat_dim % task.feat_in_channels == 0
        conv_layers = ConvBNReLU(out_channels, kernel_sizes, strides, in_channels=task.feat_in_channels) if out_channels is not None else None
        in_size = task.feat_dim // task.feat_in_channels
        if conv_layers is not None:
            in_size = conv_layers.output_feat_dim(in_size)
        else:
            in_size = task.feat_dim
        vocab = len(task.target_dictionary) if task.target_dictionary is not None else None
        encoder = cls.build_encoder(cfg, pre_encoder=conv_layers, input_size=in_size, vocab_size=vocab)
        return cls(cfg, encoder)

    @classmethod
    def build_encoder(cls, cfg, pre_encoder=None, input_size=83, vocab_size=None):
        return SpeechTransformerEncoderForPrediction(cfg, pre_encoder=pre_encoder, input_size=input_size, vocab_size=vocab_size)

    def set_num_updates(self, num_updates):
        self.num_updates = num_updates
        self.encoder.set_num_updates(num_updates)

    def early_update_modules(self):
        return self.encoder.early_modules()

    def defer_update(self, pending):
        self.encoder.pending_update = pending

    def state_dict(self, *args, **kwargs):
        if self.encoder.pending_update is not None:
            dev = next(self.parameters()).device
            self.encoder.pending_update.wait(torch.cuda.current_stream(dev))
            self.encoder.pending_update = None
        return super().state_dict(*args, **kwargs)

    def forward(self, src_tokens, src_lengths, **kwargs):
        return self.encoder(src_tokens, src_lengths, **kwargs)

    def output_lengths(self, in_lengths):
        return self.encoder.output_lengths(in_lengths)

    def max_positions(self):
        return self.encoder.max_positions()

    def get_normalized_probs(self, net_output, log_probs, sample=None):
        lg = net_output.get("_logits_bt")
        if lg:
            logits = lg[0]
            B, Tp = net_output["encoder_padding_mask"][0].shape
        else:
            e = net_output["encoder_out"][0]
            Tp, B, V = e.shape
            logits = e.transpose(0, 1).reshape(B * Tp, V)
        M, V = logits.shape
        lp = K.log_softmax(logits.detach(), M, V, logits.stride(0))
        if not log_probs:
            lp = lp.exp_()
        return lp.view(B, Tp, V).transpose(0, 1)

    def get_targets(self, sample, net_output):
        return sample["target"]

    def upgrade_state_dict_named(self, state_dict, name):
        for k in list(state_dict.keys()):
            if "conv_layers_before" in k:
                state_dict[k.replace("conv_layers_before", "pre_encoder")] = state_dict.pop(k)
        for k in list(state_dict.keys()):
            if k.endswith("positional_embedding._float_tensor") or k.endswith("embed_positions._float_tensor"):
                state_dict.pop(k)
        return state_dict


@register_model_architecture("speech_transformer_encoder_model", "speech_transformer_encoder_model")
def base_architecture(cfg):
    return cfg


@register_model_architecture("speech_transformer_encoder_model", "speech_conformer_encoder_model_librispeech")
def conformer_ctc_librispeech(cfg=None):
    cfg = cfg or SpeechTransformerConfig()
    e = cfg.encoder
    e.embed_dim, e.ffn_embed_dim, e.layers, e.attention_heads = 512, 2048, 12, 8
    e.normalize_before, e.learned_pos, e.relative_positional_embeddings = True, False, True
    e.layer_type = "conformer"
    cfg.attention_dropout = cfg.activation_dropout = cfg.dropout = 0.1
    cfg.activation_fn = "relu"
    cfg.layernorm_embedding = True
    cfg.max_source_positions, cfg.max_target_positions = 3600, 200
    return cfg
```

espresso_amd/modules/speech_convolutions.py:

```python
import torch
import torch.nn as nn

from .. import functional as F
from .params import BatchNormParams, ConvParams


class ConvBNReLU(nn.Module):
    def __init__(self, out_channels, kernel_sizes, strides, in_channels=1, apply_batchnorm=True):
        super().__init__()
        assert apply_batchnorm, "the MI355X path implements the recipes' BatchNorm variant"
        assert in_channels == 1, "fbank input has one channel (task.feat_in_channels == 1)"
        self.out_channels, self.kernel_sizes, self.strides, self.in_channels = out_channels, kernel_sizes, strides, in_channels
        self.convolutions = nn.ModuleList()
        self.batchnorms = nn.ModuleList()
        for i, co in enumerate(out_channels):
            ks = kernel_sizes[i]
            ks = tuple(ks) if isinstance(ks, (list, tuple)) else (ks, ks)
            assert ks == (3, 3), "3x3 kernels (all recipes)"
            self.convolutions.append(ConvParams(in_channels if i == 0 else out_channels[i - 1], co, ks))
            self.batchnorms.append(BatchNormParams(co))

    def _stride2(self, s):
        if isinstance(s, (list, tuple)):
            return (s[0], s[1] if len(s) > 1 else s[0])
        return (s, s)

    def output_lengths(self, in_lengths):
        out = in_lengths
        if isinstance(out, torch.Tensor):
            total = 1
            for stride in self.strides:
                total *= self._stride2(stride)[0]
            return out if total == 1 else torch.div(out + (total - 1), total, rounding_mode="floor")
        for stride in self.strides:
            s = self._stride2(stride)[0]
            if isinstance(out, torch.Tensor):
                out = torch.div(out + s - 1, s, rounding_mode="floor")
            else:
                out = (out + s - 1) // s
        return out

    def output_feat_dim(self, feat_dim):
        f = feat_dim
        for stride in self.strides:
            s = self._stride2(stride)[1]
            f = (f + s - 1) // s
        return f * self.out_channels[-1]

    def forward(self, src, src_lengths, p_drop=0.0):
        B, T, _ = src.shape
        x_lengths = self.output_lengths(src_lengths)
        Tp = (T + 0)
        for stride in self.strides:
            s = self._stride2(stride)[0]
            Tp = (Tp + s - 1) // s
        padding_mask = torch.arange(Tp, device=src.device).unsqueeze(0) >= x_lengths.unsqueeze(1)
        row_zero = padding_mask.reshape(-1).to(torch.uint8).contiguous()
        params, bufs = [], []
        for conv, bn in zip(self.convolutions, self.batchnorms):
            params += [conv.weight, conv.bias, bn.weight, bn.bias]
            bufs += [bn.running_mean, bn.running_var]
        x = F.conv_subsample(src.contiguous().float(), row_zero, [self._stride2(s) for s in self.strides], params, bufs,
                             p_drop=p_drop, training=self.training, bn_eps=self.batchnorms[0].eps,
                             bn_momentum=self.batchnorms[0].momentum, after_first_layer=getattr(self, "after_first_layer", None))
        if self.training and not getattr(self, "_counters_managed", False):
            for bn in self.batchnorms:
                bn.num_batches_tracked += 1
        return x, x_lengths, padding_mask, row_zero
```

espresso_amd/trainer.py:

```python
import contextlib

import torch
import torch.distributed as dist

from . import functional as F
from .distributed.overlapped_ddp import OverlappedDistributedDataParallel
from .optim.adam import FlatAdam
from .optim.flat import FlatParams
from .optim.noam_lr_scheduler import NoamSchedule


def grad_norms_inconsistent(norms: torch.Tensor) -> torch.Tensor:
    g0 = norms[0]
    close = ((norms - g0).abs().max() / (g0 + 1e-6)) < 1e-6
    all_bad = (~torch.isfinite(norms)).all()
    return (~(close | all_bad)).to(torch.float32).reshape(1)


class Trainer:
    def __init__(self, task, model, criterion, device, clip_norm=2.0, lr=5.0, warmup_steps=25000, adam_betas=(0.9, 0.98),
                 adam_eps=1e-8, weight_decay=0.0, final_lr=1e-6, seed=1, bucket_mb=64.0, lr_scheduler=None, defer_update=True):
        self.task, self.criterion, self.device = task, criterion, device
        self.model = model.to(device)
        self._flat = FlatParams(self.model, device)
        self._optimizer = FlatAdam(self._flat, lr=lr, betas=adam_betas, eps=adam_eps, weight_decay=weight_decay)
        if lr_scheduler is None:
            self.lr_scheduler = NoamSchedule(self._optimizer, lr=lr, warmup_steps=warmup_steps,
                                             model_size=model.cfg.encoder.embed_dim, final_lr=final_lr)
        else:
            from . import registry
            from .optim import lr_schedulers

            name, kw = lr_scheduler
            self.lr_scheduler = registry.LR_SCHEDULER_REGISTRY[name](self._optimizer, lr=lr, **kw)
        self.cfg = None
        self._optim_history = []
        self.world_size = dist.get_world_size() if dist.is_initialized() else 1
        self.ddp = OverlappedDistributedDataParallel(self.model, self._flat, bucket_mb=bucket_mb)
        self.clip_norm = clip_norm
        self.seed = seed
        self.num_updates = 0
        self._stats = torch.zeros(4 + (self.world_size if self.world_size > 1 else 0), dtype=torch.float32, device=device)
        self._gnorm_mismatch = torch.zeros(1, dtype=torch.float32, device=device)
        self.last_coef = None
        self.ooms = 0
        self._train_mode_checked = False
        self._split_update = (bool(defer_update) and torch.device(device).type == "cuda" and self._flat.early_range is not None
                              and hasattr(self.model, "defer_update"))
        self._pending_update = None

    @property
    def flat(self):
        self.flush_update()
        return self._flat

    @property
    def optimizer(self):
        self.flush_update()
        return self._optimizer

    def flush_update(self):
        pending, self._pending_update = self._pending_update, None
        if pending is not None:
            pending.wait(torch.cuda.current_stream(self._flat.p32.device))
            if hasattr(self.model, "defer_update"):
                self.model.defer_update(None)

    def train_step(self, samples):
        F.set_dropout_seed(self.seed + self.num_updates)
        if not self._split_update:
            self.flush_update()
        if not self.model.training or not self._train_mode_checked:
            self.model.train()
            self._train_mode_checked = True
        self._stats.zero_()
        F.begin_step(self._stats.device)
        for i, sample in enumerate(samples):
            last = i == len(samples) - 1
            ctx = contextlib.nullcontext() if last else self.ddp.no_sync()
            dummy = bool(sample.get("_dummy", False))
            try:
                with ctx:
                    sample = self.task.prepare_sample(sample, train=True)
                    loss, sample_size, log = self.criterion(self.ddp, sample)
                    if dummy:
                        loss = loss * 0.0
                    with F.accumulating_backward():
                        loss.backward()
            except RuntimeError as e:
                if "out of memory" not in str(e).lower():
                    raise
                self._recover_from_oom(e)
                return None
            if dummy:
                continue
            self._stats[0:1].add_(float(sample_size))
            self._stats[1:2].add_(loss.detach().reshape(1))
            self._stats[2:3].add_(float(log["ntokens"]))
            self._stats[3:4].add_(float(log["nsentences"]))
        if self.ddp.active:
            if self.world_size > 1 and self.last_coef is not None:
                self._stats[4 + dist.get_rank():5 + dist.get_rank()].copy_(self.last_coef[1:2])
            dist.all_reduce(self._stats)
            if self.world_size > 1 and self.last_coef is not None:
                self._gnorm_mismatch += grad_norms_inconsistent(self._stats[4:])
        self.ddp.all_reduce_grads()
        F.end_step()
        if self._split_update:
            self.last_coef, self._pending_update = self._optimizer.clip_and_step_split(
                F._side_stream(self._flat.p32.device), pre_scale=1.0, max_norm=self.clip_norm, denom_dev=self._stats[0:1], hold=True)
            self.model.defer_update(self._pending_update)
        else:
            self.last_coef = self._optimizer.clip_and_step(pre_scale=1.0, max_norm=self.clip_norm, denom_dev=self._stats[0:1])
        self.num_updates += 1
        if hasattr(self.model, "set_num_updates"):
            self.model.set_num_updates(self.num_updates)
        self.lr_scheduler.step_update(self.num_updates)
        return self._stats[:4]

    def _recover_from_oom(self, exc):
        import sys

        self.ooms += 1
        print(f"| WARNING: ran out of memory in the forward/backward pass of update {self.num_updates + 1} ({exc}); "
              f"{'skipping the update' if self.world_size == 1 else 'cannot skip on one rank of ' + str(self.world_size)}", file=sys.stderr)
        if self.world_size > 1:
            raise RuntimeError("out of memory on one data-parallel rank: gradient buckets of this update may already be in flight, "
                               "the update cannot be skipped consistently (lower max_tokens / batch_size)") from exc
        F.end_step()
        for m in self.model.modules():
            b = getattr(m, "_ea_binding", None)
            if b is not None:
                b.saved_busy = False
            m.__dict__.pop("_ea_chain_in", None)
            m.__dict__.pop("_ea_wt_fresh", None)
        self.flush_update()
        self._flat.zero_grad()
        self._stats.zero_()
        if self._stats.is_cuda:
            torch.cuda.synchronize(self._stats.device)
            torch.cuda.empty_cache()

    def check_grad_norm_consistency(self):
        bad = float(self._gnorm_mismatch)
        self._gnorm_mismatch.zero_()
        if bad > 0:
            raise FloatingPointError(
                f"Fatal error: gradients are inconsistent between workers ({int(bad)} update(s) since the last check). "
                "Try --ddp-backend=legacy_ddp. Or are you mixing up different generation of GPUs in training?")

    def reserve(self, samples):
        self.flush_update()
        bn = {n: b.clone() for n, b in self.model.named_buffers()}
        self.model.train()
        with self.ddp.no_sync():
            for sample in samples:
                sample = self.task.prepare_sample(sample, train=True)
                loss, _, _ = self.criterion(self.ddp, sample)
                with F.accumulating_backward():
                    loss.backward()
        self._flat.zero_grad()
        with torch.no_grad():
            for n, b in self.model.named_buffers():
                b.copy_(bn[n])
        if torch.cuda.is_available():
            torch.cuda.synchronize()

    def valid_step(self, sample):
        self.flush_update()
        return self.task.valid_step(sample, self.model, self.criterion)


    @classmethod
    def from_cfg(cls, cfg, task, model, criterion, device):
        from .config import as_list, literal

        opt, optim = cfg["optimization"], cfg["optimizer"]
        if optim.get("_name", "adam") != "adam":
            raise NotImplementedError(f"optimizer {optim.get('_name')!r} (every ASR recipe of the reference uses adam)")
        sched = dict(cfg["lr_scheduler"])
        name = sched.pop("_name")
        sched.pop("lr", None)
        if name in ("reduce_lr_on_plateau_v2", "reduce_lr_on_plateau"):
            sched.setdefault("maximize_best_checkpoint_metric", cfg["checkpoint"]["maximize_best_checkpoint_metric"])
        if name == "tri_stage":
            sched.setdefault("max_update", opt["max_update"])
            if sched.get("phase_ratio") is not None:
                sched["phase_ratio"] = literal(sched["phase_ratio"])
        t = cls(task, model, criterion, device, clip_norm=float(opt["clip_norm"]), lr=float(as_list(opt["lr"])[0]),
                adam_betas=tuple(literal(optim["adam_betas"])), adam_eps=float(optim["adam_eps"]),
                weight_decay=float(optim["weight_decay"]), seed=int(cfg["common"]["seed"]), lr_scheduler=(name, sched))
        t.cfg = cfg
        return t

    def get_lr(self):
        return self._optimizer.get_lr()

    def lr_step_begin_epoch(self, epoch):
        if hasattr(self.lr_scheduler, "step_begin_epoch"):
            self.lr_scheduler.step_begin_epoch(epoch)
        return self.get_lr()

    def lr_step(self, epoch, val_loss=None):
        if hasattr(self.lr_scheduler, "step"):
            self.lr_scheduler.step(epoch, val_loss)
        return self.get_lr()

    def _optimizer_state(self):
        self.flush_update()
        f, o = self._flat, self._optimizer
        state, ids = {}, []
        for i, p in enumerate(q for q in self.model.parameters() if q.requires_grad):
            off, n = f.offsets[id(p)], p.numel()
            state[i] = {"step": o.step_count, "exp_avg": o.exp_avg[off:off + n].view(p.shape).clone().cpu(),
                        "exp_avg_sq": o.exp_avg_sq[off:off + n].view(p.shape).clone().cpu()}
            ids.append(i)
        group = {"lr": o.lr, "betas": tuple(o.betas), "eps": o.eps, "weight_decay": o.weight_decay, "amsgrad": False, "params": ids}
        return {"state": state, "param_groups": [group]}

    def _load_optimizer_state(self, sd):
        self.flush_update()
        f, o = self._flat, self._optimizer
        params = [q for q in self.model.parameters() if q.requires_grad]
        if len(sd["state"]) not in (0, len(params)):
            raise ValueError(f"optimizer state holds {len(sd['state'])} parameters, the model has {len(params)}")
        for i, p in enumerate(params):
            st = sd["state"].get(i)
            if st is None:
                continue
            off, n = f.offsets[id(p)], p.numel()
            o.exp_avg[off:off + n].copy_(st["exp_avg"].reshape(-1))
            o.exp_avg_sq[off:off + n].copy_(st["exp_avg_sq"].reshape(-1))
            o.step_count = int(st["step"])
        if sd.get("param_groups"):
            o.lr = sd["param_groups"][0].get("lr", o.lr)

    def state_dict(self, extra_state=None):
        self.flush_update()
        sched = self.lr_scheduler.state_dict() if hasattr(self.lr_scheduler, "state_dict") else {}
        extra = {"previous_training_time": 0.0}
        extra.update(extra_state or {})
        no_optim = bool(((self.cfg or {}).get("checkpoint") or {}).get("no_save_optimizer_state", False))
        sd = {
            "args": None,
            "cfg": self.cfg,
            "model": {k: v.detach().clone().cpu() for k, v in self.model.state_dict().items()},
            "criterion": None,
            "optimizer_history": self._optim_history + [{
                "criterion_name": type(self.criterion).__name__, "optimizer_name": type(self._optimizer).__name__,
                "lr_scheduler_state": sched, "num_updates": self.num_updates}],
            "task_state": {},
            "extra_state": extra,
# ... 49 lines not shown
```

include/espresso_amd.h:

```cpp
#ifndef ESPRESSO_AMD_H
#define ESPRESSO_AMD_H

#include <stdint.h>

#ifdef __cplusplus
extern "C" {
#endif

typedef struct ihipStream_t* ea_stream_t;

int ea_version(void);

enum { EA_ACT_NONE = 0, EA_ACT_RELU = 1, EA_ACT_SILU = 2 };

typedef struct EaGemmParams {
  const void* A;
  const void* B;
  void* C;
  void* C2;
  const float* bias;
  const void* resid;
  const void* aux;
  int M, N, K, batch, zdiv;
  int a_kstrided, b_kstrided, c_f32, accumulate, resid_f32, act;
  long lda, ldb, ldc, ldc2, ldr, ldaux;
  long sA_hi, sA_lo, sB_hi, sB_lo, sC_hi, sC_lo, sR_hi, sR_lo, sX_hi, sX_lo;
  float alpha, out_scale;
  uint64_t drop_seed;
  uint32_t drop_thr;
  float drop_scale;
  int splitk, kchunk;
  void* workspace;
  void* q_u;
  void* q_v;
  const float* pos_u;
  const float* pos_v;
  long ld_q;
  int qsplit_n;
  float qscale;
} EaGemmParams;

int ea_gemm_bf16(const EaGemmParams* p, ea_stream_t stream);
long ea_gemm_splitk_workspace_bytes(int M, int N, int batch, int splitk);
int ea_set_gemm_variant(int v);
int ea_set_gemm_xcd_swizzle(int mask);
int ea_set_gemm_glds(int stages);
long ea_set_gemm_nt_store_min_bytes(long bytes);
int ea_set_gemm_w8(int mode);
int ea_gemm_profile_enable(int on);
long ea_gemm_profile_read(double* total_ms, double* total_flops);
int ea_gemm_profile_bytes(double* total_bytes);
long ea_gemm_profile_dump(const char* path);

#define EA_WGRAD_MAX 16
typedef struct EaWgradProblem {
  const void* dy;
  const void* x;
  float* dW;
  float* dbias;
  int M, N, K;
  long ld_dy, ld_x, ldw;
} EaWgradProblem;
typedef struct EaWgradGroup {
  int count;
  EaWgradProblem p[EA_WGRAD_MAX];
} EaWgradGroup;
int ea_wgrad_group(const EaWgradGroup* group, ea_stream_t stream);
int ea_set_wgrad_transposing_reads(int on);
int ea_set_wgrad_w8(int mode);

int ea_layernorm_fwd(const void* x, const float* gamma, const float* beta, void* y, float* mean, float* rstd,
                     int M, int C, float eps, const uint8_t* row_zero, uint64_t drop_seed, uint32_t drop_thr,
                     float drop_scale, ea_stream_t stream);
int ea_layernorm_fwd_f32out(const void* x, const float* gamma, const float* beta, float* y, float* mean, float* rstd,
                            int M, int C, float eps, const uint8_t* row_zero, uint64_t drop_seed, uint32_t drop_thr,
                            float drop_scale, ea_stream_t stream);
int ea_layernorm_bwd_f32dy(const void* x, const float* dy, const float* gamma, const float* mean, const float* rstd,
                           void* dx, float* dgamma, float* dbeta, int M, int C, const uint8_t* row_zero,
                           uint64_t drop_seed, uint32_t drop_thr, float drop_scale, const void* dx_add,
                           void* workspace, ea_stream_t stream);
long ea_layernorm_bwd_workspace_bytes(int M, int C);
int ea_layernorm_bwd(const void* x, const void* dy, const float* gamma, const float* mean, const float* rstd,
                     void* dx, float* dgamma, float* dbeta, int M, int C, const uint8_t* row_zero,
                     uint64_t drop_seed, uint32_t drop_thr, float drop_scale, const void* dx_add,
                     void* workspace, ea_stream_t stream);
int ea_layernorm_bwd_dx(const void* x, const void* dy, const float* gamma, const float* mean, const float* rstd, void* dx,
                        float* dgamma, float* dbeta, int M, int C, const uint8_t* row_zero, uint64_t drop_seed,
                        uint32_t drop_thr, float drop_scale, const void* dx_add, void* workspace, ea_stream_t stream);
int ea_layernorm_param_reduce(const void* workspace, float* dgamma, float* dbeta, int M, int C, ea_stream_t stream);
#define EA_LNRED_MAX 8
typedef struct EaLnReduceItem { const void* workspace; float* dgamma; float* dbeta; int M, C; } EaLnReduceItem;
typedef struct EaLnReduceGroup { int count; EaLnReduceItem item[EA_LNRED_MAX]; } EaLnReduceGroup;
int ea_layernorm_param_reduce_group(const EaLnReduceGroup* group, ea_stream_t stream);
int ea_layernorm_bwd_dx2(const void* x, const void* dy, const float* gamma, const float* mean, const float* rstd, void* dx,
                         float* dgamma, float* dbeta, int M, int C, const void* dx_add, void* workspace, void* out2, float a2,
                         uint64_t seed2, uint32_t thr2, float scale2, ea_stream_t stream);
int ea_layernorm_fwd2(const void* x, const float* g1, const float* b1, void* y1, float* mean1, float* rstd1, const float* g2,
                      const float* b2, void* y2, float* mean2, float* rstd2, int M, int C, float eps, ea_stream_t stream);
int ea_layernorm_bwd2_dx(const void* x1, const void* dy1, const float* gamma1, const float* mean1, const float* rstd1,
                         const void* dx_add, void* ws1, const void* x2, const float* gamma2, const float* mean2, const float* rstd2,
                         void* ws2, void* dx, int M, int C, void* out2, float a2, uint64_t seed2, uint32_t thr2, float scale2,
                         ea_stream_t stream);

int ea_cast_f32_to_bf16(const float* src, void* dst, long n, ea_stream_t stream);
int ea_transpose_bf16_batch(const void* const* src, void* const* dst, const int* rows, const int* cols, int n, ea_stream_t stream);
int ea_audio_probe(const char* path, long* num_samples, int* sample_rate, int* channels, int* bits);
long ea_audio_read_i16(const char* path, int16_t* dst, long capacity, int* sample_rate);
int ea_audio_verify(const char* path);
int ea_audio_read_batch_i16(const char* const* paths, int n, int16_t* dst, const long* offsets, int num_threads, long* lengths,
                            int* sample_rates);

int ea_cast_f32_to_bf16_rows(const float* src, long ld_src, void* dst, long ld_dst, long M, int N, ea_stream_t stream);
int ea_cast_bf16_to_f32(const void* src, float* dst, long n, ea_stream_t stream);
int ea_scale_dropout_bf16(const void* x, const void* y, void* out, long n, float a, float b, uint64_t seed,
                          uint32_t thr, float inv_keep, ea_stream_t stream);
int ea_colsum_bf16(const void* X, float* out, int M, int N, long ld, ea_stream_t stream);
int ea_embedding_fwd(const int* tokens, const int* positions, const float* W, const float* pos_table, void* out, int M,
                     int C, float scale, ea_stream_t stream);
int ea_embedding_bwd(const int* tokens, const void* dy, float* dW, int M, int C, float scale, int pad_idx,
                     ea_stream_t stream);
int ea_zero_rows_bf16(void* x, const uint8_t* row_zero, int M, int C, ea_stream_t stream);

int ea_flash_attention_supported(int dh, int T, int S, int relpos);
int ea_flash_attention_fwd(const void* qu, const void* qv, long ldq, const void* k, const void* v, long ldkv,
                           const void* pp, long ldpp, const int* key_len, void* out, long ldo, float* lse, int H, int B,
                           int T, int S, int dh, int causal, uint64_t drop_seed, uint32_t drop_thr, float drop_scale,
                           void* keep_bits, ea_stream_t stream);
long ea_flash_keep_bits_bytes(int H, int B, int T);
int ea_set_flash_relpos(int on);
int ea_flash_keep_bits(void* keep_bits, int H, int B, int T, uint64_t drop_seed, uint32_t drop_thr, ea_stream_t stream);
int ea_flash_attention_bwd(const void* qu, const void* qv, long ldq, const void* k, const void* v, long ldkv,
                           const void* pp, long ldpp, const int* key_len, const void* out, const void* dout, long ldo,
                           const float* lse, float* D, void* t1, void* t2, long ldt, void* dBD, int ld_bd, void* dk,
                           void* dv, long lddkv, int H, int B, int T, int S, int dh, int causal, float scaling,
                           uint64_t drop_seed, uint32_t drop_thr, float drop_scale, const void* keep_bits,
                           void* dq, long lddq, ea_stream_t stream);

int ea_relpos_q_prep(const void* qkv, long ldq, const float* u, const float* v, void* qu, void* qv, int M,
                     int C, float scaling, ea_stream_t stream);
int ea_relpos_softmax_fwd(const float* ac, const float* bd, const int* key_len, const float* attn_mask, void* P,
                          void* Pd, int H, int B, int T, int S, int ld_ac, int ld_bd, int ld_p, int causal,
                          uint64_t drop_seed, uint32_t drop_thr, float drop_scale, ea_stream_t stream);
int ea_relpos_softmax_bwd(const void* P, const float* dPd, void* dAC, void* dBD, int H, int B, int T, int S,
                          int ld_p, int ld_dp, int ld_bd, uint64_t drop_seed, uint32_t drop_thr,
                          float drop_scale, ea_stream_t stream);
int ea_add2_strided_bf16(const void* a, long lda, const void* b, long ldb, void* out, long ldo, int M, int C,
                         ea_stream_t stream);

int ea_glu_dwconv_fwd(const void* Y, const float* w, void* U, void* Z, double* stats, int B, int T, int C, int KW,
                      ea_stream_t stream);
int ea_bn_finalize(const double* stats, float* mean_rstd, float* running_mean, float* running_var, int C, float n,
                   float eps, float momentum, ea_stream_t stream);
int ea_bn_from_running(const float* running_mean, const float* running_var, float* mean_rstd, int C, float eps,
                       ea_stream_t stream);
int ea_bn_act_fwd(const void* Z, const float* mean_rstd, const float* gamma, const float* beta, void* H, long M,
                  int C, int act, ea_stream_t stream);
int ea_bn_act_bwd(const void* Z, const void* dH, const float* mean_rstd, const float* gamma, const float* beta,
                  float* red, void* dZ, float* dgamma, float* dbeta, long M, int C, int act, int training,
                  ea_stream_t stream);
long ea_dwconv_wgrad_workspace_bytes(int B, int T, int C, int KW);
int ea_glu_dwconv_bwd(const void* dZ, const void* Y, const void* U, const float* w, void* dY, float* dw,
                      void* wgrad_ws, int B, int T, int C, int KW, ea_stream_t stream);
int ea_dwconv_bwd_weight(const void* dZ, const void* U, float* dw, void* wgrad_ws, int B, int T, int C, int KW, ea_stream_t stream);
int ea_glu_dwconv_causal_fwd(const void* Y, const float* w, void* U, void* Z, double* stats, int B, int T, int C, int KW,
                             ea_stream_t stream);
int ea_glu_dwconv_causal_bwd(const void* dZ, const void* Y, const void* U, const float* w, void* dY, float* dw,
                             void* wgrad_ws, int B, int T, int C, int KW, ea_stream_t stream);
int ea_dwconv_causal_bwd_weight(const void* dZ, const void* U, float* dw, void* wgrad_ws, int B, int T, int C, int KW,
                                ea_stream_t stream);
int ea_bn_act_fwd_train(const void* Z, const double* stats, float* mean_rstd, float* running_mean, float* running_var,
                        const float* gamma, const float* beta, void* H, long M, int C, int act, float n, float eps,
                        float momentum, double* zero_next, int zero_n, ea_stream_t stream);
int ea_bn_act_bwd_fused(const void* Z, const void* dH, const float* mean_rstd, const float* gamma, const float* beta,
                        float* red, void* dZ, float* dgamma, float* dbeta, long M, int C, int act, int training,
                        float* zero_next, int zero_n, ea_stream_t stream);
int ea_bn_param_grad(const float* red, float* dgamma, float* dbeta, int C, ea_stream_t stream);
int ea_conv1_bn_bwd(const float* X, const void* Z, const void* dH, const float* mean_rstd, const float* gamma, const float* beta,
                    float* red, float* dgamma, float* dbeta, float* dW, float* dbias, int B, int T, int F, int CO, int sy, int sx,
                    int act, int training, ea_stream_t stream);

int ea_conv1_fwd(const float* X, const float* W, const float* bias, void* Z, double* stats, int B, int T, int F,
                 int CO, int sy, int sx, ea_stream_t stream);
int ea_conv1_wgrad(const float* X, const void* dZ, float* dW, float* dbias, int B, int T, int F, int CO, int sy,
                   int sx, ea_stream_t stream);
int ea_conv3x3_fwd(const void* X, const void* W, const float* bias, void* Z, double* stats, int B, int T, int F, int Cin,
                   int Cout, int sy, int sx, ea_stream_t stream);
int ea_conv3x3_dgrad(const void* dZ, const void* Wd, void* dX, int B, int T, int F, int Cin, int Cout, int sy, int sx,
                     ea_stream_t stream);
long ea_conv3x3_wgrad_workspace_bytes(int B, int T, int F, int Cin, int Cout, int sy, int sx);
int ea_conv3x3_wgrad(const void* X, const void* dZ, float* dW, void* workspace, int B, int T, int F, int Cin, int Cout, int sy,
                     int sx, ea_stream_t stream);
int ea_conv3x3_wgrad_param_layout(const void* X, const void* dZ, float* dW, void* workspace, int B, int T, int F, int Cin, int Cout,
                                  int sy, int sx, ea_stream_t stream);
int ea_im2col3x3(const void* A, void* col, int B, int T, int F, int C, int sy, int sx, ea_stream_t stream);
int ea_col2im3x3(const void* dcol, void* dA, int B, int T, int F, int C, int sy, int sx, ea_stream_t stream);
int ea_colstats_bf16(const void* X, double* stats, long M, int C, ea_stream_t stream);

int ea_log_softmax_f32(const float* in, long ld_in, float* out, long M, int V, ea_stream_t stream);
int ea_log_softmax_bf16(const void* in, long ld_in, float* out, long M, int V, ea_stream_t stream);
long ea_ctc_workspace_bytes(int B, int T, int Lmax);
int ea_ctc_loss(const float* lprobs, const int* targets, const int* in_len, const int* tgt_len, float* nll,
                void* workspace, int B, int T, int V, int Lmax, int blank, ea_stream_t stream);
int ea_ctc_grad(const float* lprobs, const void* workspace, const float* nll, const int* targets,
                const int* in_len, const int* tgt_len, void* dlogits, long ld_out, int dlogits_bf16, int B, int T,
                int V, int Lmax, int blank, float grad_scale, const float* grad_scale_dev, int zero_infinity,
                ea_stream_t stream);
int ea_ctc_greedy_decode(const void* x, long ld, int x_bf16, const int* in_len, int* best, float* bestv, int* tokens,
                         int* align, int* out_len, float* score, int B, int T, int V, int blank, int pad,
                         ea_stream_t stream);
long ea_ctc_prefix_beam_workspace_bytes(int B, int T, int beam);
int ea_ctc_prefix_beam_step(const void* x, long ld, int x_bf16, const int* in_len, void* workspace, const float* lm_rows,
                            long ld_lm, int* lm_parent, int* lm_token, void* lm_keep, int B, int T, int V, int beam, int K,
                            int blank, float lm_weight, float ins_bonus, int t0, int t1, ea_stream_t stream);
int ea_ctc_prefix_beam_finish(void* workspace, const float* lm_rows, long ld_lm, float lm_weight, float ins_bonus, int eos,
                              int B, int T, int beam, int nbest, int pad, int* tokens, int* lengths, float* scores, int* nhyp,
                              ea_stream_t stream);
long ea_ctc_prefix_beam_bias_workspace_bytes(int B, int T, int beam);
int ea_ctc_prefix_beam_bias_step(const void* x, long ld, int x_bf16, const int* in_len, void* workspace, const float* lm_rows,
                                 long ld_lm, int* lm_parent, int* lm_token, void* lm_keep, const int* cg_nodes,
                                 const int* cg_edges, const int* cg_root, int cg_n_nodes, int cg_n_edges, int B, int T, int V,
                                 int beam, int K, int blank, float lm_weight, float ins_bonus, int t0, int t1, ea_stream_t stream);
int ea_ctc_prefix_beam_bias_finish(void* workspace, const float* lm_rows, long ld_lm, float lm_weight, float ins_bonus, int eos,
                                   const int* cg_nodes, int cg_n_nodes, int B, int T, int beam, int nbest, int pad, int* tokens,
                                   int* lengths, float* scores, int* nhyp, ea_stream_t stream);
int ea_context_graph_score_host(const int* nodes_host, const int* edges_host, const int* root_host, int n_nodes, int n_edges,
                                int V, const int* tokens_host, const int* lens_host, int N, int L, float* running_host,
                                float* final_host, int* q_host);
int ea_context_graph_score(const int* nodes, const int* edges, const int* root, int n_nodes, int n_edges, int V,
                           const int* tokens, const int* lens, int N, int L, float* running, float* final_bias, int* q_out,
                           ea_stream_t stream);
long ea_ctc_prefix_beam_stream_state_bytes(int max_frames, int beam);
int ea_ctc_prefix_beam_stream_reset(void* state, const int* slots, int n, int max_streams, int max_frames, int beam,
                                    ea_stream_t stream);
int ea_ctc_prefix_beam_stream_step(const void* x, long ld, int x_bf16, long total_rows, const int* slot_idx, const int* n_new,
                                   const int* row_off, int j0, int j1, int n, void* state, const float* lm_rows, long ld_lm,
                                   int* lm_parent, int* lm_token, void* lm_keep, const int* cg_nodes, const int* cg_edges,
                                   const int* cg_root, int cg_n_nodes, int cg_n_edges, int max_streams, int max_frames, int V,
                                   int beam, int K, int blank, float lm_weight, float ins_bonus, ea_stream_t stream);
int ea_ctc_prefix_beam_stream_finish(const void* state, const int* slots, int n, const float* lm_rows, long ld_lm, float lm_weight,
                                     float ins_bonus, int eos, const int* cg_nodes, int cg_n_nodes, int max_streams,
                                     int max_frames, int beam, int nbest, int pad, int max_u, int* tokens, int* lengths,
                                     float* scores, int* nhyp, ea_stream_t stream);
int ea_ctc_prefix_beam_stream_partial(const void* state, const int* slots, int n, float lm_weight, float ins_bonus, int biased,
                                      int max_streams, int max_frames, int beam, int pad, int max_u, int* tokens, int* lengths,
                                      float* scores, int* stable_len, ea_stream_t stream);
long ea_ctc_prefix_beam_times_workspace_bytes(int B, int T, int beam);
int ea_ctc_prefix_beam_times_step(const void* x, long ld, int x_bf16, const int* in_len, void* workspace, void* times_workspace,
                                  const float* lm_rows, long ld_lm, int* lm_parent, int* lm_token, void* lm_keep,
                                  const int* cg_nodes, const int* cg_edges, const int* cg_root, int cg_n_nodes, int cg_n_edges,
                                  int B, int T, int V, int beam, int K, int blank, float lm_weight, float ins_bonus, int t0, int t1,
                                  ea_stream_t stream);
int ea_ctc_prefix_beam_times_finish(void* workspace, const void* times_workspace, const float* lm_rows, long ld_lm, float lm_weight,
                                    float ins_bonus, int eos, const int* cg_nodes, int cg_n_nodes, int B, int T, int beam,
                                    int nbest, int pad, int* tokens, int* lengths, float* scores, int* nhyp, int* times,
                                    float* vscores, ea_stream_t stream);
long ea_ctc_prefix_beam_stream_times_state_bytes(int max_frames, int beam);
int ea_ctc_prefix_beam_stream_times_reset(void* state, void* times_state, const int* slots, int n, int max_streams, int max_frames,
                                          int beam, ea_stream_t stream);
int ea_ctc_prefix_beam_stream_times_step(const void* x, long ld, int x_bf16, long total_rows, const int* slot_idx, const int* n_new,
                                         const int* row_off, int j0, int j1, int n, void* state, void* times_state,
                                         const float* lm_rows, long ld_lm, int* lm_parent, int* lm_token, void* lm_keep,
                                         const int* cg_nodes, const int* cg_edges, const int* cg_root, int cg_n_nodes,
                                         int cg_n_edges, int max_streams, int max_frames, int V, int beam, int K, int blank,
                                         float lm_weight, float ins_bonus, ea_stream_t stream);
int ea_ctc_prefix_beam_stream_times_finish(const void* state, const void* times_state, const int* slots, int n, const float* lm_rows,
                                           long ld_lm, float lm_weight, float ins_bonus, int eos, const int* cg_nodes,
                                           int cg_n_nodes, int max_streams, int max_frames, int beam, int nbest, int pad, int max_u,
                                           int* tokens, int* lengths, float* scores, int* nhyp, int* times, float* vscores,
                                           ea_stream_t stream);
int ea_ctc_prefix_beam_stream_endpoint(const void* state, const void* times_state, const int* slots, int n, float lm_weight,
                                       float ins_bonus, int biased, int max_streams, int max_frames, int beam, int silence_frames,
                                       int empty_frames, int segment_frames, int* out, ea_stream_t stream);
long ea_rnnt_frame_beam_workspace_bytes(int B, int T, int beam);
int ea_rnnt_frame_beam_step(const float* logits, long ld, const float* lm_rows, long ld_lm, int lm_no_blank, const int* in_len,
                            void* workspace, int* parent, int* token, void* keep, int B, int T, int V, int beam, int K, int blank,
                            int eos, float temperature, float lm_weight, int t, ea_stream_t stream);
int ea_rnnt_frame_beam_finish(void* workspace, int B, int T, int beam, int nbest, int pad, int normalize, int* tokens,
                              int* lengths, float* scores, int* nhyp, ea_stream_t stream);
long ea_rnnt_frame_beam_stream_state_bytes(int max_frames, int beam);
int ea_rnnt_frame_beam_stream_reset(void* state, const int* slots, int n, int max_streams, int max_frames, int beam,
                                    ea_stream_t stream);
int ea_rnnt_frame_beam_stream_step(const float* logits, long ld, const float* lm_rows, long ld_lm, int lm_no_blank,
                                   const int* slot_idx, const int* n_new, int j, int n, void* state, int* parent, int* token,
                                   void* keep, int max_streams, int max_frames, int V, int beam, int K, int blank, int eos,
                                   float temperature, float lm_weight, ea_stream_t stream);
int ea_rnnt_frame_beam_stream_finish(const void* state, const int* slots, int n, int max_streams, int max_frames, int beam,
                                     int nbest, int pad, int normalize, int max_u, int* tokens, int* lengths, float* scores,
                                     int* nhyp, ea_stream_t stream);
int ea_rnnt_frame_beam_stream_partial(const void* state, const int* slots, int n, int max_streams, int max_frames, int beam,
                                      int pad, int max_u, int* tokens, int* lengths, float* scores, int* stable_len,
                                      ea_stream_t stream);
long ea_rnnt_frame_beam_bias_workspace_bytes(int B, int T, int beam);
int ea_rnnt_frame_beam_bias_step(const float* logits, long ld, const float* lm_rows, long ld_lm, int lm_no_blank, const int* in_len,
                                 void* workspace, int* parent, int* token, void* keep, const int* cg_nodes, const int* cg_edges,
                                 const int* cg_root, int cg_n_nodes, int cg_n_edges, int B, int T, int V, int beam, int K, int blank,
                                 int eos, float temperature, float lm_weight, int t, ea_stream_t stream);
int ea_rnnt_frame_beam_bias_finish(void* workspace, const int* cg_nodes, int cg_n_nodes, int B, int T, int beam, int nbest, int pad,
                                   int normalize, int* tokens, int* lengths, float* scores, int* nhyp, ea_stream_t stream);
long ea_rnnt_frame_beam_stream_bias_state_bytes(int max_frames, int beam);
int ea_rnnt_frame_beam_stream_bias_reset(void* state, const int* slots, int n, int max_streams, int max_frames, int beam,
                                         ea_stream_t stream);
int ea_rnnt_frame_beam_stream_bias_step(const float* logits, long ld, const float* lm_rows, long ld_lm, int lm_no_blank,
                                        const int* slot_idx, const int* n_new, int j, int n, void* state, int* parent, int* token,
                                        void* keep, const int* cg_nodes, const int* cg_edges, const int* cg_root, int cg_n_nodes,
                                        int cg_n_edges, int max_streams, int max_frames, int V, int beam, int K, int blank, int eos,
                                        float temperature, float lm_weight, ea_stream_t stream);
int ea_rnnt_frame_beam_stream_bias_finish(const void* state, const int* slots, int n, int max_streams, int max_frames, int beam,
                                          const int* cg_nodes, int cg_n_nodes, int nbest, int pad, int normalize, int max_u,
                                          int* tokens, int* lengths, float* scores, int* nhyp, ea_stream_t stream);
int ea_rnnt_frame_beam_stream_bias_partial(const void* state, const int* slots, int n, int max_streams, int max_frames, int beam,
                                           int pad, int max_u, int* tokens, int* lengths, float* scores, int* stable_len,
                                           ea_stream_t stream);
long ea_rnnt_frame_beam_times_workspace_bytes(int B, int T, int beam);
int ea_rnnt_frame_beam_times_step(const float* logits, long ld, const float* lm_rows, long ld_lm, int lm_no_blank, const int* in_len,
                                  void* workspace, void* times_workspace, int* parent, int* token, void* keep, const int* cg_nodes,
                                  const int* cg_edges, const int* cg_root, int cg_n_nodes, int cg_n_edges, int B, int T, int V,
                                  int beam, int K, int blank, int eos, float temperature, float lm_weight, int t, ea_stream_t stream);
int ea_rnnt_frame_beam_times_finish(void* workspace, const void* times_workspace, const int* cg_nodes, int cg_n_nodes, int B, int T,
                                    int beam, int nbest, int pad, int normalize, int* tokens, int* lengths, float* scores, int* nhyp,
                                    int* times, float* vscores, ea_stream_t stream);
long ea_rnnt_frame_beam_stream_times_state_bytes(int max_frames, int beam);
int ea_rnnt_frame_beam_stream_times_reset(void* state, void* times_state, const int* slots, int n, int biased, int max_streams,
                                          int max_frames, int beam, ea_stream_t stream);
int ea_rnnt_frame_beam_stream_times_step(const float* logits, long ld, const float* lm_rows, long ld_lm, int lm_no_blank,
                                         const int* slot_idx, const int* n_new, int j, int n, void* state, void* times_state,
                                         int* parent, int* token, void* keep, const int* cg_nodes, const int* cg_edges,
                                         const int* cg_root, int cg_n_nodes, int cg_n_edges, int max_streams, int max_frames, int V,
                                         int beam, int K, int blank, int eos, float temperature, float lm_weight, ea_stream_t stream);
int ea_rnnt_frame_beam_stream_times_finish(const void* state, const void* times_state, const int* slots, int n, int max_streams,
                                           int max_frames, int beam, const int* cg_nodes, int cg_n_nodes, int nbest, int pad,
                                           int normalize, int max_u, int* tokens, int* lengths, float* scores, int* nhyp, int* times,
                                           float* vscores, ea_stream_t stream);
int ea_rnnt_frame_beam_stream_endpoint(const void* state, const void* times_state, const int* slots, int n, int biased,
                                       int max_streams, int max_frames, int beam, int silence_frames, int empty_frames,
                                       int segment_frames, int* out, ea_stream_t stream);
int ea_ngram_create(const char* path, void* handle_host, char* err_host, long err_cap);
int ea_ngram_destroy(void* handle);
int ea_ngram_info(const void* handle, int* meta_host, long* counts_host);
long ea_ngram_vocab(const void* handle, char* buf_host, long cap);
long ea_ngram_records(const void* handle, int order, int* ngrams_host, float* logp_host, float* bow_host);
int ea_ngram_upload(void* handle);
int ea_ngram_score_host(const void* handle, const int* ctx_host, const int* words_host, int N, float* out_host);
int ea_ngram_score(const void* handle, const int* ctx, const int* words, int N, float* out, ea_stream_t stream);
long ea_ctc_lexicon_beam_workspace_bytes(int B, int T, int beam);
int ea_ctc_lexicon_beam_search(const void* x, long ld, int x_bf16, const int* in_len, void* workspace, const void* ngram,
                               const int* trie_off, const int* trie_tok, const int* trie_child, const int* trie_word,
                               const float* trie_smear, const void* word_start, int space, int B, int T, int V, int beam, int K,
                               int blank, float lm_weight, float word_score, float ins_bonus, int nbest, int pad, int* tokens,
                               int* lengths, float* scores, int* nhyp, ea_stream_t stream);
long ea_ctc_lexicon_stream_state_bytes(int max_frames, int beam);
int ea_ctc_lexicon_stream_reset(void* state, const int* slots, int n, const void* ngram, int max_streams, int max_frames,
                                int beam, ea_stream_t stream);
int ea_ctc_lexicon_stream_step(const void* x, long ld, int x_bf16, long total_rows, const int* slot_idx, const int* n_new,
                               const int* row_off, int n, void* state, const void* ngram, const int* trie_off,
                               const int* trie_tok, const int* trie_child, const int* trie_word, const float* trie_smear,
// ... 269 lines not shown
```

Measured before the change: 5.466 audio-hours/sec.

## Fuse small tensor ops into custom kernels and add pre-transposed dgrad weights

```diff
diff --git a/espresso_amd/criterions/ctc_loss.py b/espresso_amd/criterions/ctc_loss.py
--- a/espresso_amd/criterions/ctc_loss.py
+++ b/espresso_amd/criterions/ctc_loss.py
@@ -3,7 +3,15 @@
 import torch
 
 from .. import functional as F
+from .. import kernels as K
 from ..registry import register_criterion
+
+
+def targets_and_lengths(target, pad_idx, eos_idx):
+    if target.is_cuda and target.dtype == torch.int64 and target.dim() == 2:
+        return K.ctc_targets(target.contiguous(), pad_idx, eos_idx)
+    pad_mask = (target != pad_idx) & (target != eos_idx)
+    return target.to(torch.int32).contiguous(), pad_mask.sum(-1).to(torch.int32).contiguous()
 
 
 @register_criterion("ctc_loss")
@@ -38,8 +46,9 @@
         net_output = model(**sample["net_input"], **({"epoch": self.epoch} if False else {}))
         input_lengths = net_output["src_lengths"][0]
         target = sample["target"]
-        pad_mask = (target != self.pad_idx) & (target != self.eos_idx)
-        target_lengths = pad_mask.sum(-1)
+        targets32, target_lengths = targets_and_lengths(target, self.pad_idx, self.eos_idx)
+        lens32 = net_output.get("_src_lengths_i32")
+        in_len32 = lens32[0] if lens32 and lens32[0] is not None else input_lengths.to(torch.int32).contiguous()
         lg = net_output.get("_logits_bt")
         if lg:
             logits = lg[0]
@@ -48,11 +57,8 @@
             e = net_output["encoder_out"][0]
             Tp, B, V = e.shape
             logits = e.transpose(0, 1).reshape(B * Tp, V)
-        nll, lprobs = F.ctc_loss(logits, target.to(torch.int32).contiguous(), input_lengths.to(torch.int32).contiguous(),
-                                 target_lengths.to(torch.int32).contiguous(), B, Tp, blank=self.blank_idx,
-                                 zero_infinity=self.zero_infinity)
-        if self.zero_infinity:
-            nll = torch.where(torch.isinf(nll), torch.zeros_like(nll), nll)
+        nll, lprobs = F.ctc_loss(logits, targets32, in_len32, target_lengths, B, Tp,
+                                 blank=self.blank_idx, zero_infinity=self.zero_infinity, clean=self.zero_infinity)
         loss = nll.sum()
         ntokens = sample["ntokens"] if "ntokens" in sample else int(target_lengths.sum())
         nsentences = target.size(0)
diff --git a/espresso_amd/csrc/elementwise.hip b/espresso_amd/csrc/elementwise.hip
--- a/espresso_amd/csrc/elementwise.hip
+++ b/espresso_amd/csrc/elementwise.hip
@@ -150,6 +150,74 @@
   for (int c = (threadIdx.x & 63); c < C; c += 64) atomicAdd(w + c, scale * bf2f(dy[(long)row * C + c]));
 }
 
+__global__ __launch_bounds__(256) void subsample_lengths_kernel(const long* __restrict__ src_len, long* __restrict__ x_len,
+                                                                int* __restrict__ key_len, uint8_t* __restrict__ pad_mask,
+                                                                uint8_t* __restrict__ row_zero, int B, int Tp, long total) {
+  const long i = (long)blockIdx.x * 256 + threadIdx.x;
+  auto out_len = [&](int b) {
+    const long a = src_len[b] + (total - 1);
+    long q = a / total;
+    if ((a % total != 0) && ((a < 0) != (total < 0))) --q;
+    return q;
+  };
+  if (i < B) {
+    const long q = out_len((int)i);
+    x_len[i] = q;
+    key_len[i] = (int)q;
+  }
+  if (i < (long)B * Tp) {
+    const int b = (int)(i / Tp), t = (int)(i % Tp);
+    const uint8_t m = (long)t >= out_len(b) ? 1 : 0;
+    pad_mask[i] = m;
+    row_zero[i] = m;
+  }
+}
+__global__ void stats_add4_kernel(float* __restrict__ stats, float a0, const float* __restrict__ loss, float a2, float a3) {
+  const int i = threadIdx.x;
+  if (i >= 4) return;
+  const float v = i == 0 ? a0 : i == 1 ? loss[0] : i == 2 ? a2 : a3;
+  stats[i] = stats[i] + v;
+}
+__global__ __launch_bounds__(256) void transpose_pad_kernel(const bf16_t* __restrict__ src, bf16_t* __restrict__ dst, int R, int Cc,
+                                                            long ld_dst) {
+  __shared__ bf16_t tile[64][66];
+  const int r0 = blockIdx.y * 64, c0 = blockIdx.x * 64;
+  const int tx = threadIdx.x & 63, ty = threadIdx.x >> 6;
+  for (int i = ty; i < 64; i += 4)
+    if (r0 + i < R && c0 + tx < Cc) tile[i][tx] = src[(long)(r0 + i) * Cc + c0 + tx];
+  __syncthreads();
+  for (int i = ty; i < 64; i += 4)
+    if (c0 + i < Cc && r0 + tx < ld_dst) dst[(long)(c0 + i) * ld_dst + r0 + tx] = r0 + tx < R ? tile[tx][i] : (bf16_t)0;
+}
+__global__ __launch_bounds__(256) void permute_k_kernel(const bf16_t* __restrict__ src, bf16_t* __restrict__ dst,
+                                                        bf16_t* __restrict__ dst_t, int N, int C, int F) {
+  __shared__ bf16_t tile[64][66];
+  const int CF = C * F;
+  const int r0 = blockIdx.y * 64, c0 = blockIdx.x * 64;
+  const int tx = threadIdx.x & 63, ty = threadIdx.x >> 6;
+  const int j = c0 + tx;
+  const int f = j / C, c = j % C;
+  for (int i = ty; i < 64; i += 4)
+    if (r0 + i < N && j < CF) {
+      const bf16_t v = src[(long)(r0 + i) * CF + (long)c * F + f];
+      tile[i][tx] = v;
+      dst[(long)(r0 + i) * CF + j] = v;
+    }
+  if (!dst_t) return;
+  __syncthreads();
+  for (int i = ty; i < 64; i += 4)
+    if (c0 + i < CF && r0 + tx < N) dst_t[(long)(c0 + i) * N + r0 + tx] = tile[tx][i];
+}
+__global__ __launch_bounds__(256) void unpermute_k_add_kernel(const float* __restrict__ src, float* __restrict__ dst, long n, int C, int F) {
+  const int CF = C * F;
+  for (long i = (long)blockIdx.x * 256 + threadIdx.x; i < n; i += (long)gridDim.x * 256) {
+    const long row = i / CF;
+    const int j = (int)(i % CF), f = j / C, c = j % C;
+    float* d = dst + row * CF + (long)c * F + f;
+    *d = *d + src[i];
+  }
+}
+
 }
 
 static inline int grid_for(long n, int per_thread) {
@@ -206,6 +274,39 @@
   return EA_CHECK_LAUNCH();
 }
 
+extern "C" int ea_subsample_lengths(const long* src_len, long* x_len, int* key_len, void* pad_mask, void* row_zero, int B, int Tp,
+                                    int total, hipStream_t stream) {
+  if (B <= 0) return 0;
+  if (Tp < 0 || total < 1) return -2;
+  const long n = (long)B * Tp > B ? (long)B * Tp : B;
+  hipLaunchKernelGGL(subsample_lengths_kernel, dim3((unsigned)((n + 255) / 256)), dim3(256), 0, stream, src_len, x_len, key_len,
+                     (uint8_t*)pad_mask, (uint8_t*)row_zero, B, Tp, (long)total);
+  return EA_CHECK_LAUNCH();
+}
+extern "C" int ea_stats_add4(float* stats, float a0, const float* loss, float a2, float a3, hipStream_t stream) {
+  hipLaunchKernelGGL(stats_add4_kernel, dim3(1), dim3(64), 0, stream, stats, a0, loss, a2, a3);
+  return EA_CHECK_LAUNCH();
+}
+extern "C" int ea_transpose_pad_bf16(const void* src, void* dst, int rows, int cols, long ld_dst, hipStream_t stream) {
+  if (rows <= 0 || cols <= 0) return 0;
+  if (ld_dst < rows) return -2;
+  hipLaunchKernelGGL(transpose_pad_kernel, dim3((cols + 63) / 64, (unsigned)((ld_dst + 63) / 64)), dim3(256), 0, stream,
+                     (const bf16_t*)src, (bf16_t*)dst, rows, cols, ld_dst);
+  return EA_CHECK_LAUNCH();
+}
+extern "C" int ea_permute_k_bf16(const void* src, void* dst, void* dst_t, int N, int C, int F, hipStream_t stream) {
+  if (N <= 0 || C <= 0 || F <= 0) return 0;
+  hipLaunchKernelGGL(permute_k_kernel, dim3((C * F + 63) / 64, (N + 63) / 64), dim3(256), 0, stream, (const bf16_t*)src, (bf16_t*)dst,
+                     (bf16_t*)dst_t, N, C, F);
+  return EA_CHECK_LAUNCH();
+}
+extern "C" int ea_unpermute_k_add_f32(const float* src, float* dst, int N, int C, int F, hipStream_t stream) {
+  if (N <= 0 || C <= 0 || F <= 0) return 0;
+  const long n = (long)N * C * F;
+  hipLaunchKernelGGL(unpermute_k_add_kernel, dim3(grid_for(n, 2)), dim3(256), 0, stream, src, dst, n, C, F);
+  return EA_CHECK_LAUNCH();
+}
+
 extern "C" int ea_cast_f32_to_bf16(const float* src, void* dst, long n, hipStream_t stream) {
   if (n <= 0) return 0;
   hipLaunchKernelGGL(cast_f32_bf16_kernel, dim3(grid_for(n, 8)), dim3(256), 0, stream, src, (bf16_t*)dst, n);
diff --git a/espresso_amd/csrc/loss.hip b/espresso_amd/csrc/loss.hip
--- a/espresso_amd/csrc/loss.hip
+++ b/espresso_amd/csrc/loss.hip
@@ -15,6 +15,20 @@
 }
 
 __device__ __forceinline__ int ctc_label(const int* tg, int s, int blank) { return (s & 1) ? tg[s >> 1] : blank; }
+
+__global__ __launch_bounds__(64) void ctc_targets_kernel(const long* __restrict__ target, int* __restrict__ tgt32,
+                                                         int* __restrict__ tgt_len, int L, long pad, long eos) {
+  const int b = blockIdx.x;
+  const long* tg = target + (long)b * L;
+  int cnt = 0;
+  for (int l = threadIdx.x; l < L; l += 64) {
+    const long v = tg[l];
+    tgt32[(long)b * L + l] = (int)v;
+    cnt += (v != pad && v != eos) ? 1 : 0;
+  }
+  for (int off = 32; off > 0; off >>= 1) cnt += __shfl_down(cnt, off, 64);
+  if (threadIdx.x == 0) tgt_len[b] = cnt;
+}
 
 __global__ __launch_bounds__(256) void ctc_gather_kernel(const float* __restrict__ lprobs, const int* __restrict__ targets,
                                                          const int* __restrict__ in_len, const int* __restrict__ tgt_len,
@@ -31,7 +45,7 @@
 __global__ void ctc_scan_kernel(const float* __restrict__ G, const int* __restrict__ targets,
                                 const int* __restrict__ in_len, const int* __restrict__ tgt_len,
                                 float* __restrict__ A, float* __restrict__ Bt, float* __restrict__ nll_out,
-                                int T, int Lmax, int blank, int SP) {
+                                float* __restrict__ nll_clean, int T, int Lmax, int blank, int SP) {
   extern __shared__ float sh[];
   const int b = blockIdx.x;
   const int Tb = in_len[b], L = tgt_len[b];
@@ -42,7 +56,10 @@
   float* buf1 = sh + 1 * (SP + 2) + (dir ? 0 : 2);
   const int* tg = targets + (long)b * Lmax;
   if (Tb <= 0) {
-    if (threadIdx.x == 0 && dir == 0) nll_out[b] = (L == 0) ? 0.f : INFINITY;
+    if (threadIdx.x == 0 && dir == 0) {
+      nll_out[b] = (L == 0) ? 0.f : INFINITY;
+      if (nll_clean) nll_clean[b] = 0.f;
+    }
     return;
   }
   bool skip = false;
@@ -111,7 +128,9 @@
     const float l1 = rd[S - 1];
     const float l2 = S >= 2 ? rd[S - 2] : -INFINITY;
     const float m = fmaxf(l1, l2);
-    nll_out[b] = (m == -INFINITY) ? INFINITY : -(m + logf(expf(l1 - m) + expf(l2 - m)));
+    const float v = (m == -INFINITY) ? INFINITY : -(m + logf(expf(l1 - m) + expf(l2 - m)));
+    nll_out[b] = v;
+    if (nll_clean) nll_clean[b] = (v == INFINITY || v == -INFINITY) ? 0.f : v;
   }
 }
 
@@ -329,9 +348,16 @@
   return 3L * B * T * (2L * Lmax + 1) * (long)sizeof(float);
 }
 
-extern "C" int ea_ctc_loss(const float* lprobs, const int* targets, const int* in_len, const int* tgt_len,
-                           float* nll , void* workspace, int B, int T, int V, int Lmax, int blank,
-                           hipStream_t stream) {
+extern "C" int ea_ctc_targets(const long* target, int* tgt32, int* tgt_len, int B, int L, int pad, int eos, hipStream_t stream) {
+  if (B <= 0) return 0;
+  if (L < 0) return -2;
+  hipLaunchKernelGGL(ctc_targets_kernel, dim3(B), dim3(64), 0, stream, target, tgt32, tgt_len, L, (long)pad, (long)eos);
+  return EA_CHECK_LAUNCH();
+}
+
+extern "C" int ea_ctc_loss_clean(const float* lprobs, const int* targets, const int* in_len, const int* tgt_len,
+                                 float* nll , float* nll_clean , void* workspace, int B, int T, int V,
+                                 int Lmax, int blank, hipStream_t stream) {
   if (B <= 0) return 0;
   if (T <= 0 || V <= 0 || Lmax < 0) return -2;
   const int Smax = 2 * Lmax + 1;
@@ -343,8 +369,13 @@
   hipLaunchKernelGGL(ctc_gather_kernel, dim3(T, B), dim3(256), 0, stream, lprobs, targets, in_len, tgt_len, G, T, V,
                      Lmax, blank);
   hipLaunchKernelGGL(ctc_scan_kernel, dim3(B, 2), dim3(SP), (size_t)2 * (SP + 2) * sizeof(float), stream, G, targets,
-                     in_len, tgt_len, A, Bt, nll, T, Lmax, blank, SP);
-  return EA_CHECK_LAUNCH();
+                     in_len, tgt_len, A, Bt, nll, nll_clean, T, Lmax, blank, SP);
+  return EA_CHECK_LAUNCH();
+}
+extern "C" int ea_ctc_loss(const float* lprobs, const int* targets, const int* in_len, const int* tgt_len,
+                           float* nll , void* workspace, int B, int T, int V, int Lmax, int blank,
+                           hipStream_t stream) {
+  return ea_ctc_loss_clean(lprobs, targets, in_len, tgt_len, nll, nullptr, workspace, B, T, V, Lmax, blank, stream);
 }
 
 extern "C" int ea_ctc_grad(const float* lprobs, const void* workspace, const float* nll, const int* targets,
diff --git a/espresso_amd/functional.py b/espresso_amd/functional.py
--- a/espresso_amd/functional.py
+++ b/espresso_amd/functional.py
@@ -274,7 +274,7 @@
 
 class _Linear(torch.autograd.Function):
     @staticmethod
-    def forward(ctx, x, w, b, w16, out_f32):
+    def forward(ctx, x, w, b, w16, out_f32, wt_kc=None, k_perm=None):
         M, Kin = x.shape
         N = w.shape[0]
         ld = _pad8(N)
@@ -283,6 +283,7 @@
         ctx.save_for_backward(x, w16)
         ctx.has_bias = b is not None
         ctx.params = (w, b)
+        ctx.wt_kc, ctx.k_perm = wt_kc, k_perm
         return buf if ld == N else buf[:, :N]
 
     @staticmethod
@@ -290,47 +291,92 @@
         x, w16 = ctx.saved_tensors
         M, Kin = x.shape
         N = w16.shape[0]
+        zero_pad = getattr(dy, "_ea_zero_pad", 0)
         if dy.dtype != torch.bfloat16:
+            zero_pad = 0
             if dy.stride(1) != 1:
                 dy = dy.contiguous()
             dy = K.cast_f32_to_bf16_rows(dy, _pad8(N)) if M <= 65535 else K.cast_f32_to_bf16(dy.contiguous())
         if dy.stride(1) != 1 or dy.stride(0) % 8 != 0:
-            dy = dy.contiguous()
+            dy, zero_pad = dy.contiguous(), 0
         ld = dy.stride(0)
         pw, pb = ctx.params
+        perm = ctx.k_perm
         sW = _grad_sink(pw, N * Kin)
         sb = _grad_sink(pb, N) if ctx.has_bias else None
         if sW is not None and (sb is not None or not ctx.has_bias):
             side = _side_stream(dy.device) if (dy.is_cuda and 2.0 * M * N * Kin >= 4e9) else None
+
+            def products():
+                if perm is None:
+                    _wgrad(dy, x, M, N, Kin, ld_dy=ld, out=sW.view(N, Kin), accumulate=True)
+                else:
+                    K.unpermute_k_add(_wgrad(dy, x, M, N, Kin, ld_dy=ld), sW, N, perm[0], perm[1])
+                if ctx.has_bias:
+                    K.colsum(dy, sb, M, N, ld)
+
             if side is not None:
                 cur = torch.cuda.current_stream(dy.device)
                 side.wait_stream(cur)
                 with torch.cuda.stream(side):
-                    _wgrad(dy, x, M, N, Kin, ld_dy=ld, out=sW.view(N, Kin), accumulate=True)
-                    if ctx.has_bias:
-                        K.colsum(dy, sb, M, N, ld)
+                    products()
                 dy.record_stream(side)
                 x.record_stream(side)
                 _side_pending[str(dy.device)] = True
             else:
-                _wgrad(dy, x, M, N, Kin, ld_dy=ld, out=sW.view(N, Kin), accumulate=True)
-                if ctx.has_bias:
-                    K.colsum(dy, sb, M, N, ld)
+                products()
             dW, db = None, None
         else:
             dW = _wgrad(dy, x, M, N, Kin, ld_dy=ld)
+            if perm is not None:
+                dW = dW.view(N, perm[1], perm[0]).permute(0, 2, 1).reshape(N, Kin)
             db = None
             if ctx.has_bias:
                 db = K.colsum(dy, _zeros_f32(N, dy), M, N, ld)
         dx = None
         if ctx.needs_input_grad[0]:
             dx = _new((M, Kin), torch.bfloat16, x)
-            K.gemm(dy, w16, dx, M, Kin, N, lda=ld, ldb=Kin, ldc=Kin, b_kstrided=True)
-        return dx, dW, db, None, None
-
-
-def linear(x, w, b=None, out_f32=False):
-    return _Linear.apply(x, w, b, bf16_weight(w), out_f32)
+            wt = ctx.wt_kc
+            if wt is not None and ld % _DGRAD_PITCH == 0 and tuple(wt.shape) == (Kin, ld) and (zero_pad == ld or ld == N):
+                K.gemm(dy, wt, dx, M, Kin, ld, lda=ld, ldb=ld, ldc=Kin)
+            else:
+                K.gemm(dy, w16, dx, M, Kin, N, lda=ld, ldb=Kin, ldc=Kin, b_kstrided=True)
+        return dx, dW, db, None, None, None, None
+
+
+_DGRAD_PITCH = 64
+
+
+def _pad_dgrad(n):
+    return (n + _DGRAD_PITCH - 1) // _DGRAD_PITCH * _DGRAD_PITCH
+
+
+def refresh_dgrad_weight(w):
+    sh = getattr(w, "_ea_bf16", None)
+    if sh is None or not sh.is_cuda or w.dim() != 2:
+        return False
+    N, Kin = w.shape
+    ldk = _pad_dgrad(N)
+    buf = w.__dict__.get("_ea_wt_kc")
+    if buf is None or tuple(buf.shape) != (Kin, ldk) or buf.device != sh.device:
+        buf = w.__dict__["_ea_wt_kc"] = torch.empty(Kin, ldk, dtype=torch.bfloat16, device=sh.device)
+    cur, side = torch.cuda.current_stream(sh.device), _side_stream(sh.device)
+    side.wait_stream(cur)
+    with torch.cuda.stream(side):
+        K.transpose_pad(sh.view(N, Kin), buf, N, Kin, ldk)
+    w.__dict__["_ea_wt_kc_fresh"] = buf
+    return True
+
+
+def linear(x, w, b=None, out_f32=False, k_perm=None):
+    w16 = bf16_weight(w)
+    wt_kc = w.__dict__.pop("_ea_wt_kc_fresh", None) if torch.is_grad_enabled() else None
+    if k_perm is not None:
+        if torch.is_grad_enabled() and x.requires_grad and w.shape[0] % _DGRAD_PITCH == 0:
+            w16, wt_kc = K.permute_k(w16.view(w.shape[0], -1), k_perm[0], k_perm[1], transposed=True)
+        else:
+            w16 = K.permute_k(w16.view(w.shape[0], -1), k_perm[0], k_perm[1])
+    return _Linear.apply(x, w, b, w16, out_f32, wt_kc, k_perm)
 
 
 class _LayerNorm(torch.autograd.Function):
@@ -608,33 +654,40 @@
 class _CTCLoss(torch.autograd.Function):
 
     @staticmethod
-    def forward(ctx, logits, targets, in_len, tgt_len, B, T, blank, zero_infinity):
+    def forward(ctx, logits, targets, in_len, tgt_len, B, T, blank, zero_infinity, clean=False):
         M, V = logits.shape
         assert M == B * T
         if logits.stride(1) != 1:
             logits = logits.contiguous()
         Lmax = targets.shape[1]
         lprobs = K.log_softmax(logits, M, V, logits.stride(0))
-        nll, ws = K.ctc_loss_fwd(lprobs, targets, in_len, tgt_len, B, T, V, Lmax, blank)
+        if clean:
+            nll, ws, out = K.ctc_loss_fwd(lprobs, targets, in_len, tgt_len, B, T, V, Lmax, blank, clean=True)
+        else:
+            nll, ws = K.ctc_loss_fwd(lprobs, targets, in_len, tgt_len, B, T, V, Lmax, blank)
+            out = nll
         ctx.save_for_backward(lprobs, ws, nll, targets, in_len, tgt_len)
         ctx.cfg = (B, T, V, Lmax, blank, zero_infinity, logits.dtype)
         ctx.mark_non_differentiable(lprobs)
-        return nll, lprobs
+        return out, lprobs
 
     @staticmethod
     def backward(ctx, dnll, _dlp):
         lprobs, ws, nll, targets, in_len, tgt_len = ctx.saved_tensors
         B, T, V, Lmax, blank, zero_infinity, dt = ctx.cfg
-        scale_dev = dnll.float().contiguous()
+        scale_dev = dnll.float()[:1].contiguous()
         bf = dt == torch.bfloat16
-        ld = _pad8(V) if bf else V
+        ld = _pad_dgrad(V) if bf else V
         dl = K.ctc_loss_grad(lprobs, ws, nll, targets, in_len, tgt_len, B, T, V, Lmax, blank, ld_out=ld, grad_bf16=bf,
                              grad_scale=1.0, grad_scale_dev=scale_dev, zero_infinity=zero_infinity)
-        return (dl if ld == V else dl[:, :V]), None, None, None, None, None, None, None
-
-
-def ctc_loss(logits, targets, in_len, tgt_len, B, T, blank=0, zero_infinity=True):
-    return _CTCLoss.apply(logits, targets, in_len, tgt_len, B, T, blank, zero_infinity)
+        g = dl if ld == V else dl[:, :V]
+        if bf:
+            g._ea_zero_pad = ld
+        return g, None, None, None, None, None, None, None, None
+
+
+def ctc_loss(logits, targets, in_len, tgt_len, B, T, blank=0, zero_infinity=True, clean=False):
+    return _CTCLoss.apply(logits, targets, in_len, tgt_len, B, T, blank, zero_infinity, clean)
 
 
 class _LabelSmoothedCE(torch.autograd.Function):
diff --git a/espresso_amd/kernels.py b/espresso_amd/kernels.py
--- a/espresso_amd/kernels.py
+++ b/espresso_amd/kernels.py
@@ -401,18 +401,71 @@
     return out
 
 
-def ctc_loss_fwd(lprobs, targets, in_len, tgt_len, B, T, V, Lmax, blank):
+def ctc_loss_fwd(lprobs, targets, in_len, tgt_len, B, T, V, Lmax, blank, clean=False):
     assert lprobs.dtype == torch.float32 and lprobs.is_contiguous()
     assert targets.dtype == torch.int32 and in_len.dtype == torch.int32 and tgt_len.dtype == torch.int32
+    assert targets.is_contiguous() and in_len.is_contiguous() and tgt_len.is_contiguous()
+    assert targets.numel() >= B * Lmax and in_len.numel() >= B and tgt_len.numel() >= B
     dev = lprobs.device
     nll = torch.empty(B, dtype=torch.float32, device=dev)
+    nll_clean = torch.empty(B, dtype=torch.float32, device=dev) if clean else None
     ws = torch.empty(int(_lib.lib().ea_ctc_workspace_bytes(B, T, Lmax)), dtype=torch.uint8, device=dev)
     check(
-        _lib.lib().ea_ctc_loss(_p(lprobs), _p(targets), _p(in_len), _p(tgt_len), _p(nll), _p(ws), B, T, V, Lmax, blank,
-                               _stream()),
-        "ea_ctc_loss",
+        _lib.lib().ea_ctc_loss_clean(_p(lprobs), _p(targets), _p(in_len), _p(tgt_len), _p(nll), _p(nll_clean), _p(ws), B, T, V,
+                                     Lmax, blank, _stream()),
+        "ea_ctc_loss_clean",
     )
-    return nll, ws
+    return (nll, ws, nll_clean) if clean else (nll, ws)
+
+
+def ctc_targets(target, pad, eos):
+    assert target.dtype == torch.int64 and target.dim() == 2 and target.is_contiguous()
+    B, L = target.shape
+    tgt32 = torch.empty(B, L, dtype=torch.int32, device=target.device)
+    tgt_len = torch.empty(B, dtype=torch.int32, device=target.device)
+    check(_lib.lib().ea_ctc_targets(_p(target), _p(tgt32), _p(tgt_len), B, L, int(pad), int(eos), _stream()), "ea_ctc_targets")
+    return tgt32, tgt_len
+
+
+def subsample_lengths(src_lengths, total, Tp):
+    assert src_lengths.dtype == torch.int64 and src_lengths.dim() == 1 and src_lengths.is_contiguous()
+    B, dev = src_lengths.numel(), src_lengths.device
+    x_len = torch.empty(B, dtype=torch.int64, device=dev)
+    key_len = torch.empty(B, dtype=torch.int32, device=dev)
+    mask = torch.empty(B, Tp, dtype=torch.bool, device=dev)
+    row_zero = torch.empty(B * Tp, dtype=torch.uint8, device=dev)
+    check(_lib.lib().ea_subsample_lengths(_p(src_lengths), _p(x_len), _p(key_len), _p(mask), _p(row_zero), B, Tp, int(total),
+                                          _stream()), "ea_subsample_lengths")
+    return x_len, key_len, mask, row_zero
+
+
+def stats_add4(stats, a0, loss, a2, a3):
+    assert stats.dtype == torch.float32 and stats.is_contiguous() and stats.numel() >= 4
+    assert loss.dtype == torch.float32 and loss.numel() == 1
+    check(_lib.lib().ea_stats_add4(_p(stats), float(a0), _p(loss), float(a2), float(a3), _stream()), "ea_stats_add4")
+    return stats
+
+
+def transpose_pad(src, dst, rows, cols, ld_dst):
+    assert src.dtype == torch.bfloat16 and dst.dtype == torch.bfloat16 and src.is_contiguous() and dst.is_contiguous()
+    assert src.numel() == rows * cols and dst.numel() == cols * ld_dst and ld_dst >= rows
+    check(_lib.lib().ea_transpose_pad_bf16(_p(src), _p(dst), rows, cols, ld_dst, _stream()), "ea_transpose_pad_bf16")
+    return dst
+
+
+def permute_k(src, C, F, transposed=False):
+    assert src.dtype == torch.bfloat16 and src.is_contiguous() and src.dim() == 2 and src.shape[1] == C * F
+    dst = torch.empty_like(src)
+    dst_t = torch.empty(C * F, src.shape[0], dtype=torch.bfloat16, device=src.device) if transposed else None
+    check(_lib.lib().ea_permute_k_bf16(_p(src), _p(dst), _p(dst_t), src.shape[0], C, F, _stream()), "ea_permute_k_bf16")
+    return (dst, dst_t) if transposed else dst
+
+
+def unpermute_k_add(src, dst, N, C, F):
+    assert src.dtype == torch.float32 and dst.dtype == torch.float32 and src.is_contiguous() and dst.is_contiguous()
+    assert src.numel() == N * C * F and dst.numel() == N * C * F
+    check(_lib.lib().ea_unpermute_k_add_f32(_p(src), _p(dst), N, C, F, _stream()), "ea_unpermute_k_add_f32")
+    return dst
 
 
 def ctc_loss_grad(lprobs, ws, nll, targets, in_len, tgt_len, B, T, V, Lmax, blank, ld_out=None, grad_bf16=True,
diff --git a/espresso_amd/models/transformer/speech_transformer_encoder_model.py b/espresso_amd/models/transformer/speech_transformer_encoder_model.py
--- a/espresso_amd/models/transformer/speech_transformer_encoder_model.py
+++ b/espresso_amd/models/transformer/speech_transformer_encoder_model.py
@@ -151,6 +151,9 @@
             table = self._sin_table
         return F.add_positions(x, table, pos, self.embed_scale)
 
+    def _refresh_output_transpose(self, train):
+        return False
+
     def _fc0_weight(self):
         w = self.fc0.weight
         C = self.pre_encoder.out_channels[-1]
@@ -167,7 +170,11 @@
         x, x_lengths, padding_mask, row_zero = self.pre_encoder(src_tokens, src_lengths, p_drop=p if self.fc0 is not None else 0.0)
         Tp = padding_mask.shape[1]
         if self.fc0 is not None:
-            x = F.linear(x, self._fc0_weight(), self.fc0.bias)
+            if x.is_cuda:
+                C0 = self.pre_encoder.out_channels[-1]
+                x = F.linear(x, self.fc0.weight, self.fc0.bias, k_perm=(C0, self.fc0.weight.shape[1] // C0))
+            else:
+                x = F.linear(x, self._fc0_weight(), self.fc0.bias)
         if self.abs_positions or self.embed_scale != 1.0:
             x = self._add_positions(x, padding_mask)
         if self.layernorm_embedding is not None:
@@ -177,16 +184,25 @@
                 x = F.dropout(x, p)
             if row_zero is not None:
                 x = F.zero_rows(x, row_zero)
-        key_len = x_lengths.to(torch.int32).contiguous()
+        key_len = getattr(self.pre_encoder, "_key_len", None)
+        if key_len is None:
+            key_len = x_lengths.to(torch.int32).contiguous()
+        self._key_len = key_len
         attn_mask = self.get_attn_mask(Tp, x.device, in_lengths=x_lengths)
         states = [x] if return_all_hiddens else []
         ld = float(getattr(cfg.encoder, "layerdrop", 0.0) or 0.0)
         keep = torch.empty(len(self.layers)).uniform_() > ld if (tr and ld > 0) else None
         wt_event = None
-        if tr and torch.is_grad_enabled() and x.is_cuda:
+        train_pass = bool(tr and torch.is_grad_enabled() and x.is_cuda)
+        if not train_pass:
+            self._refresh_output_transpose(False)
+        if train_pass:
             native = [l for i, l in enumerate(self.layers) if (keep is None or bool(keep[i])) and _native_conformer(l)]
+            out_fresh = self._refresh_output_transpose(True)
             if native:
                 wt_event = F.refresh_layer_transposes(native, B, Tp)
+            if wt_event is None and out_fresh:
+                wt_event = F._side_stream(x.device).record_event()
         if self.pending_update is not None:
             self.pending_update.wait(torch.cuda.current_stream(x.device))
             self.pending_update = None
@@ -241,6 +257,7 @@
         out["src_lengths"] = [l.index_select(0, new_order) for l in encoder_out["src_lengths"]]
         out["encoder_states"] = [s.index_select(1, new_order) for s in encoder_out["encoder_states"]]
         out.pop("_x_bt", None)
+        out.pop("_src_lengths_i32", None)
         return out
 
 
@@ -255,6 +272,15 @@
     def __init__(self, cfg, pre_encoder=None, input_size=83, vocab_size=None):
         super().__init__(cfg, pre_encoder=pre_encoder, input_size=input_size)
         self.fc_out = LinearParams(cfg.encoder.embed_dim, vocab_size) if vocab_size is not None else None
+
+    def _refresh_output_transpose(self, train):
+        if self.fc_out is None:
+            return False
+        self.fc_out.weight.__dict__.pop("_ea_wt_kc_fresh", None)
+        if not train:
+            return False
+        self.start_pending_update()
+        return F.refresh_dgrad_weight(self.fc_out.weight)
 
     def forward(self, src_tokens, src_lengths, return_all_hiddens=False):
         out = super().forward(src_tokens, src_lengths, return_all_hiddens=return_all_hiddens)
@@ -265,6 +291,7 @@
             V = logits.shape[1]
             out["encoder_out"] = [logits.view(B, Tp, V).transpose(0, 1)]
             out["_logits_bt"] = [logits]
+            out["_src_lengths_i32"] = [self._key_len]
         return out
 
 
diff --git a/espresso_amd/modules/speech_convolutions.py b/espresso_amd/modules/speech_convolutions.py
--- a/espresso_amd/modules/speech_convolutions.py
+++ b/espresso_amd/modules/speech_convolutions.py
@@ -2,6 +2,7 @@
 import torch.nn as nn
 
 from .. import functional as F
+from .. import kernels as K
 from .params import BatchNormParams, ConvParams
 
 
@@ -40,6 +41,16 @@
                 out = (out + s - 1) // s
         return out
 
+    def lengths_and_masks(self, src_lengths, Tp):
+        if src_lengths.is_cuda and src_lengths.dtype == torch.int64 and src_lengths.dim() == 1:
+            total = 1
+            for stride in self.strides:
+                total *= self._stride2(stride)[0]
+            return K.subsample_lengths(src_lengths.contiguous(), total, Tp)
+        x_lengths = self.output_lengths(src_lengths)
+        padding_mask = torch.arange(Tp, device=src_lengths.device).unsqueeze(0) >= x_lengths.unsqueeze(1)
+        return x_lengths, None, padding_mask, padding_mask.reshape(-1).to(torch.uint8).contiguous()
+
     def output_feat_dim(self, feat_dim):
         f = feat_dim
         for stride in self.strides:
@@ -49,13 +60,11 @@
 
     def forward(self, src, src_lengths, p_drop=0.0):
         B, T, _ = src.shape
-        x_lengths = self.output_lengths(src_lengths)
         Tp = (T + 0)
         for stride in self.strides:
             s = self._stride2(stride)[0]
             Tp = (Tp + s - 1) // s
-        padding_mask = torch.arange(Tp, device=src.device).unsqueeze(0) >= x_lengths.unsqueeze(1)
-        row_zero = padding_mask.reshape(-1).to(torch.uint8).contiguous()
+        x_lengths, self._key_len, padding_mask, row_zero = self.lengths_and_masks(src_lengths, Tp)
         params, bufs = [], []
         for conv, bn in zip(self.convolutions, self.batchnorms):
             params += [conv.weight, conv.bias, bn.weight, bn.bias]
diff --git a/espresso_amd/trainer.py b/espresso_amd/trainer.py
--- a/espresso_amd/trainer.py
+++ b/espresso_amd/trainer.py
@@ -4,6 +4,7 @@
 import torch.distributed as dist
 
 from . import functional as F
+from . import kernels as K
 from .distributed.overlapped_ddp import OverlappedDistributedDataParallel
 from .optim.adam import FlatAdam
 from .optim.flat import FlatParams
@@ -94,10 +95,14 @@
                 return None
             if dummy:
                 continue
-            self._stats[0:1].add_(float(sample_size))
-            self._stats[1:2].add_(loss.detach().reshape(1))
-            self._stats[2:3].add_(float(log["ntokens"]))
-            self._stats[3:4].add_(float(log["nsentences"]))
+            if self._stats.is_cuda:
+                K.stats_add4(self._stats, float(sample_size), loss.detach().reshape(1).float(), float(log["ntokens"]),
+                             float(log["nsentences"]))
+            else:
+                self._stats[0:1].add_(float(sample_size))
+                self._stats[1:2].add_(loss.detach().reshape(1))
+                self._stats[2:3].add_(float(log["ntokens"]))
+                self._stats[3:4].add_(float(log["nsentences"]))
         if self.ddp.active:
             if self.world_size > 1 and self.last_coef is not None:
                 self._stats[4 + dist.get_rank():5 + dist.get_rank()].copy_(self.last_coef[1:2])
diff --git a/include/espresso_amd.h b/include/espresso_amd.h
--- a/include/espresso_amd.h
+++ b/include/espresso_amd.h
@@ -112,6 +112,12 @@
 
 int ea_cast_f32_to_bf16_rows(const float* src, long ld_src, void* dst, long ld_dst, long M, int N, ea_stream_t stream);
 int ea_cast_bf16_to_f32(const void* src, float* dst, long n, ea_stream_t stream);
+int ea_subsample_lengths(const long* src_len, long* x_len, int* key_len, void* pad_mask, void* row_zero, int B, int Tp, int total,
+                         ea_stream_t stream);
+int ea_stats_add4(float* stats, float a0, const float* loss, float a2, float a3, ea_stream_t stream);
+int ea_transpose_pad_bf16(const void* src, void* dst, int rows, int cols, long ld_dst, ea_stream_t stream);
+int ea_permute_k_bf16(const void* src, void* dst, void* dst_t, int N, int C, int F, ea_stream_t stream);
+int ea_unpermute_k_add_f32(const float* src, float* dst, int N, int C, int F, ea_stream_t stream);
 int ea_scale_dropout_bf16(const void* x, const void* y, void* out, long n, float a, float b, uint64_t seed,
                           uint32_t thr, float inv_keep, ea_stream_t stream);
 int ea_colsum_bf16(const void* X, float* out, int M, int N, long ld, ea_stream_t stream);
@@ -201,6 +207,9 @@
 long ea_ctc_workspace_bytes(int B, int T, int Lmax);
 int ea_ctc_loss(const float* lprobs, const int* targets, const int* in_len, const int* tgt_len, float* nll,
                 void* workspace, int B, int T, int V, int Lmax, int blank, ea_stream_t stream);
+int ea_ctc_loss_clean(const float* lprobs, const int* targets, const int* in_len, const int* tgt_len, float* nll,
+                      float* nll_clean, void* workspace, int B, int T, int V, int Lmax, int blank, ea_stream_t stream);
+int ea_ctc_targets(const long* target, int* tgt32, int* tgt_len, int B, int L, int pad, int eos, ea_stream_t stream);
 int ea_ctc_grad(const float* lprobs, const void* workspace, const float* nll, const int* targets,
                 const int* in_len, const int* tgt_len, void* dlogits, long ld_out, int dlogits_bf16, int B, int T,
                 int V, int Lmax, int blank, float grad_scale, const float* grad_scale_dev, int zero_infinity,
```

Measured after the change: 5.525 audio-hours/sec, median of 6. +1.1%, better.
